# tum-vision/lsd_slam

Hardware: AMD Instinct MI355X
Metric: tracked frames/sec (full track+map loop) at 640x480, frames resident in HBM (8-bit upload excluded: value_pcie_inclusive has it) (higher is better)
Workload: dtype f32

## Files before the change

### include/lsd_slam_hip.hpp

```cpp
#ifndef LSD_SLAM_HIP_HPP
#define LSD_SLAM_HIP_HPP

#include <chrono>
#include <cmath>
#include <cstdint>
#include <cstring>
#include <deque>
#include <exception>
#include <functional>
#include <map>
#include <memory>
#include <mutex>
#include <stdexcept>
#include <string>
#include <tuple>
#include <utility>
#include <vector>

#include "lsdhip.h"

namespace lsd_slam_hip {

struct Error : std::runtime_error {
  int status;
// ... 311 lines not shown
    std::vector<SE3> out((size_t)n);
    for (int j = 0; j < n; j++) out[j] = SE3::from7(results[j].frameToReference);
    return out;
  }
  SE3 trackFrameOnPermaref(Frame* reference, Frame* frame, SE3 referenceToFrame) {
    pushSettings();
    double init[7];
    referenceToFrame.to7(init);
    lsdhip_track_result r;
    check(lsdhip_tracker_track_permaref(h_, reference->permaRef_posData.data(), reference->permaRef_colorAndVarData.data(),
                                        reference->permaRefNumPts, frame->handle(), init, &r), "lsdhip_tracker_track_permaref");
    publish(r);
    return SE3::from7(r.frameToReference);
  }
  void setEnqueueHook(std::function<void()> fn) {
    hook_ = std::move(fn);
    check(lsdhip_tracker_set_enqueue_hook(h_, hook_ ? &SE3Tracker::hookTrampoline : nullptr, this), "lsdhip_tracker_set_enqueue_hook");
  }
  float checkPermaRefOverlap(Frame* reference, SE3 referenceToFrame) {
    double init[7];
    referenceToFrame.to7(init);
    float usage = 0;
    check(lsdhip_tracker_check_overlap(h_, reference->permaRef_posData.data(), reference->permaRefNumPts, init, &usage), "lsdhip_tracker_check_overlap");
    pointUsage = usage;
    return usage;
  }

  float pointUsage = 0, lastGoodCount = 0, lastMeanRes = 0, lastBadCount = 0, lastResidual = 0;
  float affineEstimation_a = 1, affineEstimation_b = 0;
  bool diverged = false, trackingWasGood = false;
  int numEvaluations = 0, numWarpUpdates = 0;
  int levelEvaluations[LSDHIP_PYRAMID_LEVELS] = {0, 0, 0, 0, 0};
  int numLaunches = 0;
  void setSpeculation(int trials, int finestLevelWorkgroups = 0) { check(lsdhip_tracker_set_speculation(h_, trials, finestLevelWorkgroups), "lsdhip_tracker_set_speculation"); }
  void setBatchCoarseMinJobs(int minJobs) { check(lsdhip_tracker_set_batch_coarse_min_jobs(h_, minJobs), "lsdhip_tracker_set_batch_coarse_min_jobs"); }

 private:
  void pushSettings() {
    lsdhip_tracker_settings st;
    st.lambdaSuccessFac = settings.lambdaSuccessFac; st.lambdaFailFac = settings.lambdaFailFac;
    for (int l = 0; l < LSDHIP_PYRAMID_LEVELS; l++) {
      st.lambdaInitial[l] = settings.lambdaInitial[l]; st.stepSizeMin[l] = settings.stepSizeMin[l];
      st.convergenceEps[l] = settings.convergenceEps[l]; st.maxItsPerLvl[l] = settings.maxItsPerLvl[l];
    }
    st.lambdaInitialTestTrack = settings.lambdaInitialTestTrack; st.stepSizeMinTestTrack = settings.stepSizeMinTestTrack;
    st.convergenceEpsTestTrack = settings.convergenceEpsTestTrack; st.maxItsTestTrack = settings.maxItsTestTrack;
    st.huber_d = settings.huber_d; st.var_weight = settings.var_weight;
    check(lsdhip_tracker_set_settings(h_, &st), "lsdhip_tracker_set_settings");
  }
  void publish(const lsdhip_track_result& r) {
    pointUsage = r.pointUsage; lastGoodCount = r.lastGoodCount; lastMeanRes = r.lastMeanRes; lastBadCount = r.lastBadCount;
    lastResidual = r.lastResidual; affineEstimation_a = r.affineEstimation_a; affineEstimation_b = r.affineEstimation_b;
    diverged = r.diverged != 0; trackingWasGood = r.trackingWasGood != 0;
    numEvaluations = r.numEvaluations; numWarpUpdates = r.numWarpUpdates;
    int st[8];
    if (lsdhip_tracker_exec_stats(h_, st) == 0) for (int l = 0; l < LSDHIP_PYRAMID_LEVELS; l++) levelEvaluations[l] = st[3 + l];
    int ls[2];
    if (lsdhip_tracker_launch_stats(h_, ls) == 0) numLaunches = ls[0];
  }
  static void hookTrampoline(void* self) {
    SE3Tracker* t = static_cast<SE3Tracker*>(self);
    try { if (t->hook_) t->hook_(); } catch (...) { t->hookError_ = std::current_exception(); }
  }
  std::function<void()> hook_;
  std::exception_ptr hookError_;
  std::shared_ptr<Context> ctx_;
// ... 126 lines not shown
  float msUpdate = 0, msCreate = 0, msFinalize = 0, msObserve = 0, msRegularize = 0, msPropagate = 0, msFillHoles = 0, msSetDepth = 0;
  lsdhip_depthmap* handle() const { return h_; }

 private:
  void timings() {
    float t[8];
    if (lsdhip_depth_timings(h_, t) == 0) { msUpdate = t[0]; msCreate = t[1]; msFinalize = t[2]; msObserve = t[3]; msRegularize = t[4]; msPropagate = t[5]; msFillHoles = t[6]; msSetDepth = t[7]; }
  }
  std::shared_ptr<Context> ctx_;
  lsdhip_depthmap* h_ = nullptr;
};

class SlamLoop {
 public:
  SlamLoop(int w, int h, const Mat3f& K, const unsigned char* firstImage, bool imagesOnDevice, const float* gtDepth0, int kfEvery)
      : tracker(w, h, K), map(w, h, K), w_(w), h_(h), K_(K), onDevice_(imagesOnDevice), kfEvery_(kfEvery) {
    const int its[LSDHIP_PYRAMID_LEVELS] = {5, 20, 50, 100, 0};
    std::memcpy(tracker.settings.maxItsPerLvl, its, sizeof(its));
    keyframe = makeFrame(0, firstImage);
    if (gtDepth0) {
      keyframe->setDepthFromGroundTruth(gtDepth0);
      map.initializeFromGTDepth(keyframe.get());
    } else {
      map.initializeRandomly(keyframe.get());
    }
    trackKF_ = keyframe;
    reference.importFrame(keyframe.get());
    keyframe->clearDepthHasBeenUpdatedFlag();
    tracker.setEnqueueHook([this]() {
      flushDeferredMapping();
      if (!pendingNext_) return;
      prefetched_ = makeFrame(frameId_ + 1, pendingNext_, true);
      prefetchedSrc_ = pendingNext_;
    });
  }
  SlamLoop(const SlamLoop&) = delete;
  SlamLoop& operator=(const SlamLoop&) = delete;
  void setPipelined(bool on) {
    if (frameId_ != 0) throw Error(LSDHIP_E_STATE, "SlamLoop::setPipelined: switch before the first frame");
    Context::get(w_, h_, K_)->setPipeline(on);
    pipelined_ = on;
  }
  bool pipelined() const { return pipelined_; }
  void flushDeferredMapping() {
    if (!deferredMap_) return;
    std::shared_ptr<Frame> frame = std::move(deferredMap_);
    deferredMap_.reset();
    runUpdate(frame);
  }
  static float keyframeScore(float distanceSquared, float usage) {
    return distanceSquared * 4.0f * 4.0f + (1 - usage) * (1 - usage) * 3.0f * 3.0f;
  }
  std::function<void(Frame&, DepthMap&)> onKeyframeFinished;
  std::function<void(Frame&)> onKeyframeFinishedAsync;
  SE3 step(const unsigned char* image) { return step(image, [](double) {}); }
  template <typename F>
  SE3 step(const unsigned char* image, F&& onTrackEnd, const unsigned char* nextImage = nullptr) {
    if (trackingLost) throw Error(LSDHIP_E_STATE, "SlamLoop: tracking lost (no relocaliser here): create a new loop");
    lsdhip_host_mark(0);
    frameId_++;
    std::shared_ptr<Frame> frame;
    if (prefetched_ && prefetchedSrc_ == image) frame = std::move(prefetched_);
    else frame = makeFrame(frameId_, image);
    prefetched_.reset();
    pendingNext_ = nextImage;
    if (!pipelined_ && keyframe->depthHasBeenUpdatedFlag()) {
      reference.importFrame(keyframe.get());
      keyframe->clearDepthHasBeenUpdatedFlag();
    }
    lsdhip_host_mark(1);
    const std::shared_ptr<Frame> trackedOn = trackKF_;
    SE3 est = tracker.trackFrame(&reference, frame.get(), lastFrameToKF_);
    lsdhip_host_mark(8);
    pendingNext_ = nullptr;
    evaluations += tracker.numEvaluations;
    launches += tracker.numLaunches;
    for (int l = 0; l < LSDHIP_PYRAMID_LEVELS; l++) levelEvaluations[l] += tracker.levelEvaluations[l];
    if (tracker.trackingWasGood) numTrackedGood++;
    numTracked++;
    lastTrackEnd = std::chrono::duration<double>(std::chrono::steady_clock::now().time_since_epoch()).count();
    onTrackEnd(lastTrackEnd);
    if (tracker.diverged || (numKeyframesFinished_ > 5  && !tracker.trackingWasGood)) {
      trackingLost = true;
      reference.invalidate();
      if (map.isValid()) {
        if (mappedOnKF_ >= 5 ) {
          map.finalizeKeyFrame();
          numKeyframesFinished_++;
          if (onKeyframeFinished) onKeyframeFinished(*keyframe, map);
          if (onKeyframeFinishedAsync) onKeyframeFinishedAsync(*keyframe);
        }
        map.invalidate();
      }
      throw Error(LSDHIP_DIVERGED, std::string("SlamLoop: tracking lost at frame ") + std::to_string(frameId_) +
                                       (tracker.diverged ? " (diverged)" : " (trackingWasGood false)"));
    }
// ... 428 lines not shown
```

### include/lsdhip.h

```cpp
#ifndef LSDHIP_H
#define LSDHIP_H

#include <stddef.h>
#include <stdint.h>

#ifdef __cplusplus
extern "C" {
#endif

#define LSDHIP_PYRAMID_LEVELS 5

#define LSDHIP_OK 0
#define LSDHIP_DIVERGED 1
#define LSDHIP_E_ARG (-1)
#define LSDHIP_E_HIP (-2)
#define LSDHIP_E_STATE (-3)
#define LSDHIP_E_CAPACITY (-4)
#define LSDHIP_CLOUD_TABLE_FULL 2
#define LSDHIP_CLOUD_GUARD_POINTS 64

typedef struct lsdhip_ctx lsdhip_ctx;
typedef struct lsdhip_frame lsdhip_frame;
typedef struct lsdhip_tracker lsdhip_tracker;
typedef struct lsdhip_depthmap lsdhip_depthmap;
// ... 78 lines not shown
} lsdhip_track_result;

typedef struct lsdhip_residual_record {
  int warped_size;
  float goodCount, badCount, pointUsage, meanRes, retval;
  float affine_a_lastIt, affine_b_lastIt;
  float weightedError;
  float A[36], b[6], lsError;
  double num_constraints;
} lsdhip_residual_record;

int lsdhip_tracker_create(lsdhip_ctx* ctx, lsdhip_tracker** out);
void lsdhip_tracker_destroy(lsdhip_tracker* t);
int lsdhip_tracker_set_max_its(lsdhip_tracker* t, const int maxItsPerLvl[LSDHIP_PYRAMID_LEVELS]);
typedef struct lsdhip_tracker_settings {
  float lambdaSuccessFac, lambdaFailFac;
  float lambdaInitial[LSDHIP_PYRAMID_LEVELS], stepSizeMin[LSDHIP_PYRAMID_LEVELS], convergenceEps[LSDHIP_PYRAMID_LEVELS];
  int maxItsPerLvl[LSDHIP_PYRAMID_LEVELS];
  float lambdaInitialTestTrack, stepSizeMinTestTrack, convergenceEpsTestTrack, maxItsTestTrack;
  float huber_d, var_weight;
} lsdhip_tracker_settings;
int lsdhip_tracker_get_settings(const lsdhip_tracker* t, lsdhip_tracker_settings* out);
int lsdhip_tracker_set_settings(lsdhip_tracker* t, const lsdhip_tracker_settings* in);
int lsdhip_tracker_exec_stats(const lsdhip_tracker* t, int out[8]);
int lsdhip_tracker_set_speculation(lsdhip_tracker* t, int trials, int finestLevelWorkgroups);
int lsdhip_tracker_set_batch_coarse_min_jobs(lsdhip_tracker* t, int minJobs);
int lsdhip_tracker_launch_stats(const lsdhip_tracker* t, int out[2]);
int lsdhip_tracker_step_stats(const lsdhip_tracker* t, int out[4]);
int lsdhip_tracker_summary_stats(const lsdhip_tracker* t, long long out[6]);
int lsdhip_tracker_eval_throughput(lsdhip_tracker* t, int n, lsdhip_frame** keyframes, lsdhip_frame** frames, const float* refToFrame,
                                   int level, int repeats, double* ms_per_launch, double* bytes_per_launch);
typedef void (*lsdhip_enqueue_hook)(void* user);
int lsdhip_tracker_set_enqueue_hook(lsdhip_tracker* t, lsdhip_enqueue_hook fn, void* user);
int lsdhip_tracker_track(lsdhip_tracker* t, lsdhip_frame* keyframe, lsdhip_frame* frame,
                         const double frameToReference_initialEstimate[7], lsdhip_track_result* out);
int lsdhip_tracker_track_batch(lsdhip_tracker* t, int n, lsdhip_frame** keyframes, lsdhip_frame** frames,
                               const double* frameToReference_initialEstimates, lsdhip_track_result* results);
int lsdhip_tracker_evaluate(lsdhip_tracker* t, lsdhip_frame* keyframe, lsdhip_frame* frame,
                            const float referenceToFrame[7], int level, float affine_a, float affine_b,
                            lsdhip_residual_record* out);
int lsdhip_tracker_evaluate_batch(lsdhip_tracker* t, int n, lsdhip_frame** keyframes, lsdhip_frame** frames,
                                  const float* referenceToFrame, const float* affine, int level, lsdhip_residual_record* out,
                                  int* form);
int lsdhip_tracker_track_permaref(lsdhip_tracker* t, const float* pos3_host, const float* colorAndVar2_host, int n,
                                  lsdhip_frame* frame, const double referenceToFrame[7], lsdhip_track_result* out);
int lsdhip_tracker_track_permaref_batch(lsdhip_tracker* t, int n, const float* pos3_host, const float* colorAndVar2_host,
                                        const int* counts, lsdhip_frame** frames, const double* referenceToFrame,
                                        lsdhip_track_result* results);
int lsdhip_tracker_check_overlap(lsdhip_tracker* t, const float* pos3_host, int n, const double referenceToFrame[7],
                                 float* usage_out);

typedef struct lsdhip_sim3tracker lsdhip_sim3tracker;
typedef struct lsdhip_sim3_result {
  double frameToReference[8];
  float lastResidual, lastDepthResidual, lastPhotometricResidual;
  float pointUsage;
  float affineEstimation_a, affineEstimation_b;
  int diverged;
  int numEvaluations;
  float lastSim3Hessian[49];
} lsdhip_sim3_result;
typedef struct lsdhip_sim3_eval_record {
  int warped_size;
  float pointUsage, affine_a_lastIt, affine_b_lastIt;
  float sumResD, sumResP;
  int numTermsD, numTermsP;
// ... 90 lines not shown
```

### include/lsdhip_driver.h

```cpp
#ifndef LSDHIP_DRIVER_H
#define LSDHIP_DRIVER_H
#include <stdint.h>
#ifdef __cplusplus
extern "C" {
#endif
typedef struct lsdloop lsdloop;
typedef struct lsdloop_stats {
  double seconds_track;
  double seconds_map;
  double seconds_keyframe;
  long long frames;
  long long updates;
  long long keyframes;
  long long evaluations;
  long long tracked_good;
  long long level_evaluations[5];
  long long track_launches;
  long long dropped;
} lsdloop_stats;
int lsdloop_create(int device, int w, int h, const float K4[4], const uint8_t* first_image, int images_on_device,
                   const float* gt_depth0_host, int kf_every, lsdloop** out);
void lsdloop_destroy(lsdloop* l);
int lsdloop_run(lsdloop* l, const uint8_t* const* images, int n, int stop_at_keyframe, double* frameToKeyframe_out);
int lsdloop_get_stats(lsdloop* l, lsdloop_stats* out);
int lsdloop_reset_stats(lsdloop* l);
int lsdloop_copy_keyframe_planes(lsdloop* l, float* idepth_dev, float* idepthVar_dev);
int lsdloop_set_keyframe_ring(lsdloop* l, float* ring_dev, int slots);
long long lsdloop_keyframes_exported(lsdloop* l);
int lsdloop_keep_keyframes(lsdloop* l, int on);
int lsdloop_keyframe_log(lsdloop* l, double* scales_out, long long* points_out, int max);
int lsdloop_set_pipeline(lsdloop* l, int on);
int lsdloop_set_live_queue(lsdloop* l, int frames);
int lsdloop_set_speculation(lsdloop* l, int trials, int finest_level_workgroups);
int lsdloop_observe_time(lsdloop* l, double* ms_out, long long* calls_out);
int lsdloop_observe_work(lsdloop* l, double out3[3]);
int lsdloop_comm_unique_id(unsigned char out128[128]);
int lsdloop_comm_init(lsdloop* l, const unsigned char id128[128], int rank, int world);
int lsdloop_comm_destroy(lsdloop* l);
int lsdloop_gather_keyframes(lsdloop* l, int count, int root, float* recv_dev, long long stride_floats);
int lsdloop_gather_counts(lsdloop* l, int* counts_out, int cap);
int lsdloop_ipc_init(lsdloop* l, int rank, int world, int root, unsigned char handle64_out[64]);
int lsdloop_ipc_connect(lsdloop* l, const unsigned char root_handle64[64]);
int lsdloop_ipc_result(lsdloop* l, int* counts_out, float** data_out);
void* lsdloop_ctx(lsdloop* l);
typedef struct lsdloopbatch lsdloopbatch;
int lsdloopbatch_create(int device, int w, int h, const float K4[4], int S, const uint8_t* const* first_images, int images_on_device,
                        const float* const* gt_depth0_host, int kf_every, lsdloopbatch** out);
void lsdloopbatch_destroy(lsdloopbatch* l);
int lsdloopbatch_run(lsdloopbatch* l, const uint8_t* const* images, int n, double* frameToKeyframe_out);
int lsdloopbatch_get_stats(lsdloopbatch* l, long long* out6_per_sequence);
void* lsdloopbatch_ctx(lsdloopbatch* l);
int lsdloopbatch_set_keyframe_phases(lsdloopbatch* l, const int* phase);
int lsdloopbatch_set_pipeline(lsdloopbatch* l, int on);
int lsdloopbatch_set_coarse_min_jobs(lsdloopbatch* l, int min_jobs);
long long lsdloopbatch_dropped(lsdloopbatch* l, int sequence);
int lsdloopbatch_keep_keyframes(lsdloopbatch* l, int on);
// ... 32 lines not shown
```

### lsd_slam_amd/capi.py

```python
import ctypes as C
import os

import numpy as np

_HERE = os.path.dirname(os.path.abspath(__file__))
LIB_PATH = os.environ.get("LSDHIP_LIB") or os.path.join(_HERE, "liblsdhip.so")
_lib = None

HYP_DTYPE = np.dtype(
    [("isValid", np.uint8), ("_pad", np.uint8, 3), ("blacklisted", np.int32), ("nextStereoFrameMinID", np.float32),
     ("validity_counter", np.int32), ("idepth", np.float32), ("idepth_var", np.float32),
     ("idepth_smoothed", np.float32), ("idepth_var_smoothed", np.float32)])
assert HYP_DTYPE.itemsize == 32


class BuildDefaults(C.Structure):
    _fields_ = [(k, C.c_int) for k in ("ctx_async", "ctx_pipeline", "spec_trials_small", "spec_small_pixels", "spec_trials_mid", "spec_mid_pixels",
                                         "spec_workgroups", "spec_workgroups_above_pixels", "spec_trials_max", "batch_throughput_min_jobs",
                                         "batch_strip_workgroups", "batch_coarse_min_jobs", "batch_coarse_max_pixels",
                                         "batch_coarse_max_points")]


class Params(C.Structure):
    _fields_ = [("minUseGrad", C.c_float), ("cameraPixelNoise2", C.c_float), ("depthSmoothingFactor", C.c_float),
# ... 77 lines not shown
        "lsdhip_frame_set_counters": (i, [vp, i, i, i, i]),
        "lsdhip_frame_depth_updated": (i, [vp]),
        "lsdhip_frame_clear_depth_updated": (i, [vp]),
        "lsdhip_ref_pointcloud": (i, [vp, i, vp, vp, vp, vp]),
        "lsdhip_tracker_create": (i, [vp, pvp]),
        "lsdhip_tracker_destroy": (None, [vp]),
        "lsdhip_tracker_set_max_its": (i, [vp, vp]),
        "lsdhip_tracker_get_settings": (i, [vp, C.POINTER(TrackerSettings)]),
        "lsdhip_tracker_set_settings": (i, [vp, C.POINTER(TrackerSettings)]),
        "lsdhip_depth_copy_rows_batch": (i, [vp, i, vp]),
        "lsdhip_ctx_alloc_dev": (i, [vp, C.c_size_t, vp]),
        "lsdhip_ctx_ipc_export": (i, [vp, vp, vp]),
        "lsdhip_ctx_ipc_open": (i, [vp, vp, vp]),
        "lsdhip_ctx_ipc_close": (i, [vp, vp]),
        "lsdhip_ctx_flag_set": (i, [vp, vp, i]),
        "lsdhip_ctx_flag_wait": (i, [vp, vp, i, vp]),
        "lsdhip_ctx_memset_dev": (i, [vp, vp, i, C.c_size_t]),
        "lsdhip_ctx_read_dev": (i, [vp, vp, vp, C.c_size_t]),
        "lsdhip_ctx_free_dev": (i, [vp, vp]),
        "lsdhip_host_mark": (None, [i]),
        "lsdhip_ctx_aux_begin": (i, [vp]),
        "lsdhip_ctx_aux_end": (i, [vp]),
        "lsdhip_ctx_aux_join": (i, [vp]),
        "lsdhip_ctx_aux_stream": (vp, [vp]),
        "lsdhip_depth_stage_rows": (i, [vp, i, i, i, i]),
        "lsdhip_depth_stage_rows_batch": (i, [vp, i, pvp, C.POINTER(C.c_int), C.POINTER(C.c_int)]),
        "lsdhip_tracker_exec_stats": (i, [vp, vp]),
        "lsdhip_tracker_set_speculation": (i, [vp, i, i]),
        "lsdhip_tracker_set_batch_coarse_min_jobs": (i, [vp, i]),
        "lsdhip_tracker_launch_stats": (i, [vp, vp]),
        "lsdhip_tracker_summary_stats": (i, [vp, vp]),
        "lsdhip_tracker_step_stats": (i, [vp, vp]),
        "lsdhip_tracker_set_enqueue_hook": (i, [vp, vp, vp]),
        "lsdhip_tracker_track": (i, [vp, vp, vp, vp, C.POINTER(TrackResult)]),
        "lsdhip_tracker_track_batch": (i, [vp, i, pvp, pvp, vp, C.POINTER(TrackResult)]),
        "lsdhip_tracker_eval_throughput": (i, [vp, i, pvp, pvp, vp, i, i, C.POINTER(C.c_double), C.POINTER(C.c_double)]),
        "lsdhip_tracker_evaluate": (i, [vp, vp, vp, vp, i, f, f, C.POINTER(ResidualRecord)]),
        "lsdhip_tracker_evaluate_batch": (i, [vp, i, pvp, pvp, vp, vp, i, C.POINTER(ResidualRecord), vp]),
        "lsdhip_tracker_track_permaref": (i, [vp, vp, vp, i, vp, vp, C.POINTER(TrackResult)]),
        "lsdhip_tracker_track_permaref_batch": (i, [vp, i, vp, vp, vp, pvp, vp, C.POINTER(TrackResult)]),
        "lsdhip_tracker_check_overlap": (i, [vp, vp, i, vp, C.POINTER(C.c_float)]),
        "lsdhip_sim3tracker_create": (i, [vp, pvp]),
        "lsdhip_sim3tracker_destroy": (None, [vp]),
        "lsdhip_sim3tracker_set_max_its": (i, [vp, vp]),
        "lsdhip_sim3tracker_track": (i, [vp, vp, vp, vp, i, i, C.POINTER(Sim3Result)]),
        "lsdhip_sim3tracker_track_batch": (i, [vp, i, pvp, pvp, vp, i, i, C.POINTER(Sim3Result)]),
        "lsdhip_host_se3f_step": (i, [vp, vp, vp]),
        "lsdhip_host_ldlt6": (i, [vp, vp, vp]),
        "lsdhip_host_sim3_step": (i, [vp, vp, vp]),
        "lsdhip_host_ldlt7": (i, [vp, vp, vp]),
        "lsdhip_devtest_se3f_lm_step": (i, [vp, i, vp, vp, vp, vp, vp, vp]),
        "lsdhip_devtest_sim3_lm_step": (i, [vp, i, vp, vp, vp, vp, vp, vp, vp]),
        "lsdhip_sim3tracker_evaluate": (i, [vp, vp, vp, vp, i, f, f, C.POINTER(Sim3EvalRecord)]),
        "lsdhip_depth_create": (i, [vp, pvp]),
        "lsdhip_depth_destroy": (None, [vp]),
        "lsdhip_depth_is_valid": (i, [vp]),
        "lsdhip_depth_invalidate": (i, [vp]),
        "lsdhip_depth_reset": (i, [vp]),
        "lsdhip_depth_init_gt": (i, [vp, vp]),
        "lsdhip_depth_init_random": (i, [vp, vp]),
        "lsdhip_depth_set_from_existing": (i, [vp, vp]),
        "lsdhip_depth_update": (i, [vp, pvp, i]),
        "lsdhip_depth_observe_work": (i, [vp, vp]),
        "lsdhip_depth_update_batch": (i, [i, pvp, pvp]),
        "lsdhip_depth_create_keyframe": (i, [vp, vp, C.POINTER(C.c_float)]),
        "lsdhip_depth_change_keyframe_batch": (i, [i, pvp, pvp, C.POINTER(C.c_float)]),
# ... 56 lines not shown
```

### lsd_slam_amd/csrc/lsdhip_internal.hpp

```cpp
#pragma once
#include <hip/hip_runtime.h>
#include <cmath>
#include <cstddef>
#include <cstdint>
#include <cstdio>
#include <cstring>
#include <mutex>
#include <string>
#include <vector>
#include "../../include/lsdhip.h"

#define LSD_LEVELS LSDHIP_PYRAMID_LEVELS
#define LSD_TRACK_MIN_LEVEL 1
#define LSD_TRACK_MAX_LEVEL 5
#define LSD_QUICK_KF_CHECK_LVL 4

void lsd_set_error(const char* fmt, ...);
#define HIPCHK(expr)                                                                       \
  do {                                                                                     \
    hipError_t e_ = (expr);                                                                \
    if (e_ != hipSuccess) {                                                                \
      lsd_set_error("%s failed: %s (%s:%d)", #expr, hipGetErrorString(e_), __FILE__, __LINE__); \
      return LSDHIP_E_HIP;                                                                 \
    }                                                                                      \
// ... 10 lines not shown
  RS_M = 0,
  RS_GOOD, RS_BAD, RS_SUMRES2, RS_SUMSIGNED, RS_SXX, RS_SYY, RS_SX, RS_SY, RS_SW, RS_USAGE,
  RS_WERR,
  RS_A0,
  RS_B0 = RS_A0 + 21,
  RS_ERR = RS_B0 + 6,
  RS_NREF,
  RS_END,
  RS_TOP0 = RS_END
};
static_assert(RS_TOP0 + 3 <= RS_NUM, "record too small");
static_assert(RS_END <= RS_NUM, "record too small");

struct TrackLevel {
  const float* kf_idepth;
  const float* kf_idepthVar;
  const float* kf_image;
  const uint8_t* kf_refBlk;
  const float4* fr_grad;
  const float* pts_pos;
  const float* pts_colvar;
  int npts;
  int w, h;
  int nblocks;
  int singlePass;
  int tilePx;
  float fx, fy, cx, cy, fxi, fyi, cxi, cyi;
  float lambdaInitial, stepSizeMin, convergenceEps;
  int maxIts;
  float minWarped;
  int writeMask;
};

struct TrackJob {
  TrackLevel lv[LSD_LEVELS];
  uint8_t* wasGood;
  float cameraPixelNoise2, var_weight, huber_half;
  float lambdaSuccessFac, lambdaFailFac;
  int useAffine;
  int lastLevel;
  int topLevel;
  lsdm::SE3fH T0;
  float aff_a0, aff_b0;
  int evalOnly;
  int trackFrameSemantics;
};
struct TrackSpec {
  int specC;
  int specGrid;
  int trials[LSD_LEVELS];
  uint8_t* wasGoodSide;
  unsigned maskStride;
  int seq;
  int copyMask;
  unsigned long long dbgCum;
  unsigned long long* dbgCounters;
  int last;
#ifdef LSD_PHASE_TRACE
  int traceWg;
#endif
#ifdef LSD_DEVTOOLS
  int* dbgLog;
#endif
};

#define LSD_SPEC_MAX 6
struct TrackState {
  lsdm::SE3fH T;
  lsdm::SE3fH Tn;
  float R[9], t[3];
  float aff_a, aff_b, aff_a_lastIt, aff_b_lastIt;
  float lastErr, LM_lambda, last_residual;
  int level, iteration, incTry, phase;
  int pending;
  float A[36], b[6];
  float inc[6];
  float bytes;
  int done, diverged;
  int numEvaluations, numWarpUpdates;
  float pointUsage, goodCount, badCount, meanRes;
  int levelEvals[LSD_LEVELS];
  int ncand;
  int lastCand;
  int numLaunches;
};

struct TrackSummary {
  int done;
  int diverged, level, numEvaluations, numWarpUpdates, pad_[3];
  float q[4], t[3];
  float lastResidual, pointUsage, goodCount, badCount, meanRes, aff_a, aff_b, aff_a_lastIt, aff_b_lastIt;
  float sums[RS_NUM];
  double bytes;
  int levelEvals[LSD_LEVELS];
  int numLaunches;
  int lastCand;
  int seq;
  int exhausted;
  unsigned check;
};
#define LSD_SUMMARY_CHECK_WORDS (offsetof(TrackSummary, seq) / 4)
__host__ __device__ static inline unsigned lsd_summary_term(unsigned i, unsigned bits) { return bits * (2u * i + 1u); }

struct DeferredSlot { double sum, count, flag, pad; };
#define LSD_NUM_SLOTS 256
#define LSD_DEFAULT_ASYNC 0
#define LSD_DEFAULT_PIPELINE 0
#define LSD_SPEC_TRIALS_SMALL 6
#define LSD_SPEC_SMALL_PX 6144
#define LSD_SPEC_TRIALS_MID 5
#define LSD_SPEC_MID_PX 90112
#define LSD_SPEC_CAP_WORKGROUPS 80
#define LSD_SPEC_CAP_ABOVE_PX 24576
#ifndef LSD_OBS_SPLIT_MIN_MAPS
#define LSD_OBS_SPLIT_MIN_MAPS 4
#endif
#define LSD_OBS_WALK_WAVES 4096
#define LSD_BATCH_THROUGHPUT_MIN_JOBS 8
#define LSD_BATCH_SPEC_MAX 4
#define LSD_BATCH_SPEC_PIXELS 500000
#define LSD_BATCH_STRIP_WORKGROUPS 768
struct lsdhip_frame;

#define LSD_CTX_LOCK(c) std::lock_guard<std::recursive_mutex> lsd_ctx_lock_((c)->mtx)
struct lsdhip_ctx {
  std::recursive_mutex mtx;
  int device = 0;
  bool async = LSD_DEFAULT_ASYNC != 0;
  DeferredSlot* h_slots = nullptr;
// ... 136 lines not shown
  int levelEvaluations[LSD_LEVELS] = {};
  int block = 256;
  int grid_cap = 304;
  int recent[4] = {0, 0, 0, 0};
  int specC = 6;
  int soloMinJobs = -1;
  bool specAuto = true;
  int specCaps[LSD_LEVELS] = {0, 0, 0, 0, 0};
  int specLevel[LSD_LEVELS] = {0, 0, 0, 0, 0};
  int specCap = LSD_SPEC_CAP_WORKGROUPS;
  uint8_t* d_maskSide = nullptr;
  int maskSet = 0;
  long long maskMergeSeq[2] = {0, 0};
  size_t maskStride = 0;
  int numLaunches = 0;
  long long sumPolled = 0, sumLate = 0, sumLateMaxNs = 0, sumLateWords = 0;
  int sumLateFirstWord = -1, sumLateLastWord = -1;
  unsigned long long dbgCum = 0;
  std::vector<unsigned> dumpL0;
  unsigned long long* d_dbg = nullptr;
#ifdef LSD_DEVTOOLS
  int* d_log = nullptr;
  std::vector<int> lastLog;
#endif
  TrackSpec spec = {};
  const lsdhip_frame* jobKf = nullptr;
  unsigned jobKfVersion = 0;
  int jobTag = 0, launchOrdinal = 0;
  int budgetExtra = 2;
  int budgetFixed = 0;
  long long dbgJobs = 0, dbgEnqueued = 0, dbgMisses = 0, dbgWaitNs = 0, dbgLaunchNs = 0;
  TrackSummary* h_summary = nullptr;
  TrackSummary* d_summary = nullptr;
  unsigned long long* d_trace = nullptr;
  int batch_capacity = 0;
  TrackJob* d_bjobs = nullptr;
  TrackJob* h_bjobs = nullptr;
  TrackState* d_bstate = nullptr;
  float* d_bscratch = nullptr;
  int batchRecent[4] = {0, 0, 0, 0};
  int batchTag = 1;
  TrackSummary* h_bsummary = nullptr;
  float* d_pts = nullptr;
  int pts_capacity = 0;
};

#ifdef __HIP_DEVICE_COMPILE__
#define LSD_G __attribute__((address_space(1)))
#else
#define LSD_G
#endif
template <typename T> __host__ __device__ inline LSD_G T* lsd_g(T* p) { return (LSD_G T*)p; }
struct HypPlanes {
  LSD_G uint8_t* valid;
  LSD_G int32_t* blacklisted;
  LSD_G float* nextID;
  LSD_G int32_t* validity;
  LSD_G float* idepth;
  LSD_G float* var;
  LSD_G float* idepth_s;
  LSD_G float* var_s;
};

struct StereoRef {
  LSD_G const float* image;
  LSD_G const uint8_t* wasGood;
// ... 115 lines not shown
```

### lsd_slam_amd/csrc/pose_math.hpp

```cpp
#pragma once
#include <hip/hip_runtime.h>
#include <cmath>

#define LSDM_HD __host__ __device__ inline

namespace lsdm {
struct Quatd { double w, x, y, z; };
struct Quatf { float w, x, y, z; };
struct SE3dH { Quatd q; double t[3]; };
struct SE3fH { Quatf q; float t[3]; };
struct Sim3dH { Quatd q; double t[3]; double s; };

template <typename Q> LSDM_HD Q q_conj(const Q& a) { Q r = {a.w, -a.x, -a.y, -a.z}; return r; }
template <typename Q> LSDM_HD Q q_mul(const Q& a, const Q& b) {
  Q r;
  r.w = a.w * b.w - a.x * b.x - a.y * b.y - a.z * b.z;
  r.x = a.w * b.x + a.x * b.w + a.y * b.z - a.z * b.y;
  r.y = a.w * b.y + a.y * b.w + a.z * b.x - a.x * b.z;
  r.z = a.w * b.z + a.z * b.w + a.x * b.y - a.y * b.x;
  return r;
}
LSDM_HD void q_normalize(Quatf& q) {
  float n = sqrtf(q.x * q.x + q.y * q.y + q.z * q.z + q.w * q.w);
  q.w /= n; q.x /= n; q.y /= n; q.z /= n;
// ... 22 lines not shown
LSDM_HD void quatf_to_rot(const Quatf& q, float R[9]) { q_to_rot<Quatf, float>(q, R); }
LSDM_HD void quatd_to_rot(const Quatd& q, double R[9]) { q_to_rot<Quatd, double>(q, R); }

LSDM_HD SE3dH se3d_from7(const double p[7]) { SE3dH T; T.q = {p[0], p[1], p[2], p[3]}; T.t[0] = p[4]; T.t[1] = p[5]; T.t[2] = p[6]; return T; }
LSDM_HD void se3d_to7(const SE3dH& T, double p[7]) { p[0] = T.q.w; p[1] = T.q.x; p[2] = T.q.y; p[3] = T.q.z; p[4] = T.t[0]; p[5] = T.t[1]; p[6] = T.t[2]; }
LSDM_HD SE3dH se3d_inverse(const SE3dH& T) {
  SE3dH r;
  r.q = q_conj(T.q);
  double nt[3] = {T.t[0] * -1.0, T.t[1] * -1.0, T.t[2] * -1.0};
  q_rotate<Quatd, double>(r.q, nt, r.t);
  return r;
}
LSDM_HD SE3fH se3f_from_d(const SE3dH& T) {
  SE3fH r;
  r.q = {(float)T.q.w, (float)T.q.x, (float)T.q.y, (float)T.q.z};
  q_normalize(r.q);
  for (int i = 0; i < 3; i++) r.t[i] = (float)T.t[i];
  return r;
}
LSDM_HD SE3dH se3d_from_f(const SE3fH& T) {
  SE3dH r;
  r.q = {(double)T.q.w, (double)T.q.x, (double)T.q.y, (double)T.q.z};
  q_normalize(r.q);
  for (int i = 0; i < 3; i++) r.t[i] = (double)T.t[i];
  return r;
}
LSDM_HD SE3fH se3f_inverse(const SE3fH& T) {
  SE3fH r;
  r.q = q_conj(T.q);
  float nt[3] = {T.t[0] * -1.0f, T.t[1] * -1.0f, T.t[2] * -1.0f};
  q_rotate<Quatf, float>(r.q, nt, r.t);
  return r;
}
LSDM_HD SE3fH se3f_mul(const SE3fH& a, const SE3fH& b) {
  SE3fH r = a;
  float rt[3];
  q_rotate<Quatf, float>(a.q, b.t, rt);
  for (int i = 0; i < 3; i++) r.t[i] = a.t[i] + rt[i];
  r.q = q_mul(a.q, b.q);
  q_normalize(r.q);
  return r;
}
LSDM_HD SE3fH se3f_exp(const float a[6]) {
  const float eps = static_cast<float>(1e-5);
  float ox = a[3], oy = a[4], oz = a[5];
  float theta_sq = ox * ox + (oy * oy + oz * oz);
  float theta = sqrtf(theta_sq);
  float half_theta = 0.5f * theta;
  float imag, real;
  if (theta < eps) {
    float theta_po4 = theta_sq * theta_sq;
    imag = 0.5f - static_cast<float>(1.0 / 48.0) * theta_sq + static_cast<float>(1.0 / 3840.0) * theta_po4;
    real = 1.0f - 0.5f * theta_sq + static_cast<float>(1.0 / 384.0) * theta_po4;
  } else {
    float s = sinf(half_theta);
    imag = s / theta;
    real = cosf(half_theta);
  }
  SE3fH r;
  r.q = {real, imag * ox, imag * oy, imag * oz};
  q_normalize(r.q);
  float Om[9] = {0, -oz, oy, oz, 0, -ox, -oy, ox, 0};
  float Om2[9];
  for (int i = 0; i < 3; i++)
    for (int j = 0; j < 3; j++) {
      float acc = Om[i * 3 + 0] * Om[0 * 3 + j];
// ... 80 lines not shown
```

### lsd_slam_amd/csrc/track_device.hpp

```cpp
#pragma once
#include "lsdhip_internal.hpp"
#include <type_traits>

template <int CTRL, int ROW_MASK, int BANK_MASK>
__device__ __forceinline__ float dpp_f(float v) {
  return __builtin_bit_cast(float, __builtin_amdgcn_update_dpp(0, __builtin_bit_cast(int, v), CTRL, ROW_MASK, BANK_MASK, true));
}
__device__ __forceinline__ int dpp_max_i(int a, int b) { return a > b ? a : b; }
template <int CTRL, int ROW_MASK, int BANK_MASK>
__device__ __forceinline__ int dpp_i(int v) {
  return __builtin_amdgcn_update_dpp(-1, v, CTRL, ROW_MASK, BANK_MASK, false);
}
template <int CTRL, int ROW_MASK, int BANK_MASK>
__device__ __forceinline__ int dpp_i0(int v) {
  return __builtin_amdgcn_update_dpp(0, v, CTRL, ROW_MASK, BANK_MASK, true);
}
__device__ __forceinline__ int wave_max_to_lane63(int v) {
  int t = dpp_max_i(v, dpp_i<0x111, 0xf, 0xf>(v));
  t = dpp_max_i(t, dpp_i<0x112, 0xf, 0xf>(v));
  t = dpp_max_i(t, dpp_i<0x113, 0xf, 0xf>(v));
  t = dpp_max_i(t, dpp_i<0x114, 0xf, 0xe>(t));
  t = dpp_max_i(t, dpp_i<0x118, 0xf, 0xc>(t));
  t = dpp_max_i(t, dpp_i<0x142, 0xa, 0xf>(t));
  t = dpp_max_i(t, dpp_i<0x143, 0xc, 0xf>(t));
// ... 298 lines not shown
__device__ __forceinline__ lsdm::SE3fH se3f_mul_wave(const lsdm::SE3fH& a, const lsdm::SE3fH& b, const int lane) {
  lsdm::SE3fH r = a;
  float rt[3];
  lsdm::q_rotate<lsdm::Quatf, float>(a.q, b.t, rt);
#pragma unroll
  for (int i = 0; i < 3; i++) r.t[i] = a.t[i] + rt[i];
  r.q = lsdm::q_mul(a.q, b.q);
  q_normalize_wave(r.q, lane);
  return r;
}

__device__ __forceinline__ void write_summary(const TrackState& s, const float* tot, TrackSummary* out, const int doneWord) {
  unsigned chk = (unsigned)doneWord;
#define SUM_PUT_I(field, value) do { const int v_ = (value); out->field = v_; chk += lsd_summary_term((unsigned)(offsetof(TrackSummary, field) / 4), (unsigned)v_); } while (0)
#define SUM_PUT_F(field, value) do { const float v_ = (value); out->field = v_; chk += lsd_summary_term((unsigned)(offsetof(TrackSummary, field) / 4), __float_as_uint(v_)); } while (0)
#define SUM_PUT_IA(field, i, value) do { const int v_ = (value); out->field[i] = v_; chk += lsd_summary_term((unsigned)(offsetof(TrackSummary, field) / 4 + (i)), (unsigned)v_); } while (0)
#define SUM_PUT_FA(field, i, value) do { const float v_ = (value); out->field[i] = v_; chk += lsd_summary_term((unsigned)(offsetof(TrackSummary, field) / 4 + (i)), __float_as_uint(v_)); } while (0)
  SUM_PUT_I(diverged, s.diverged); SUM_PUT_I(level, s.level); SUM_PUT_I(numEvaluations, s.numEvaluations); SUM_PUT_I(numWarpUpdates, s.numWarpUpdates);
  SUM_PUT_IA(pad_, 0, 0); SUM_PUT_IA(pad_, 1, 0); SUM_PUT_IA(pad_, 2, 0);
  SUM_PUT_FA(q, 0, s.T.q.w); SUM_PUT_FA(q, 1, s.T.q.x); SUM_PUT_FA(q, 2, s.T.q.y); SUM_PUT_FA(q, 3, s.T.q.z);
  SUM_PUT_FA(t, 0, s.T.t[0]); SUM_PUT_FA(t, 1, s.T.t[1]); SUM_PUT_FA(t, 2, s.T.t[2]);
  SUM_PUT_F(lastResidual, s.last_residual); SUM_PUT_F(pointUsage, s.pointUsage); SUM_PUT_F(goodCount, s.goodCount); SUM_PUT_F(badCount, s.badCount);
  SUM_PUT_F(meanRes, s.meanRes); SUM_PUT_F(aff_a, s.aff_a); SUM_PUT_F(aff_b, s.aff_b); SUM_PUT_F(aff_a_lastIt, s.aff_a_lastIt); SUM_PUT_F(aff_b_lastIt, s.aff_b_lastIt);
  for (int i = 0; i < RS_NUM; i++) SUM_PUT_FA(sums, i, tot[i]);
  {
    const double b = (double)s.bytes;
    out->bytes = b;
    const unsigned long long u = (unsigned long long)__double_as_longlong(b);
    chk += lsd_summary_term((unsigned)(offsetof(TrackSummary, bytes) / 4), (unsigned)u) + lsd_summary_term((unsigned)(offsetof(TrackSummary, bytes) / 4 + 1), (unsigned)(u >> 32));
  }
  for (int l = 0; l < LSD_LEVELS; l++) SUM_PUT_IA(levelEvals, l, s.levelEvals[l]);
  SUM_PUT_I(numLaunches, s.numLaunches);
  SUM_PUT_I(lastCand, s.lastCand);
#undef SUM_PUT_I
#undef SUM_PUT_F
#undef SUM_PUT_IA
#undef SUM_PUT_FA
  out->check = chk;
  __threadfence_system();
  out->done = doneWord;
}

struct LmShared {
  float gj[48];
  float tot[RS_NUM];
};
struct LmPar {
  float lambdaInitial, stepSizeMin, convergenceEps, minWarped, lambdaSuccessFac, lambdaFailFac;
  int maxIts, w, h, writeMask, evalOnly, useAffine, tfSemantics, lastLevel, trials;
};
__device__ __forceinline__ void stage_lm_par(const TrackJob& job, int level, LmPar& p, const int trials = 1) {
  const TrackLevel& L = job.lv[level];
  LmPar v;
  v.lambdaInitial = L.lambdaInitial; v.stepSizeMin = L.stepSizeMin; v.convergenceEps = L.convergenceEps; v.minWarped = L.minWarped;
  v.lambdaSuccessFac = job.lambdaSuccessFac; v.lambdaFailFac = job.lambdaFailFac;
  v.maxIts = L.maxIts; v.w = L.w; v.h = L.h; v.writeMask = L.writeMask; v.evalOnly = job.evalOnly; v.useAffine = job.useAffine;
  v.tfSemantics = job.trackFrameSemantics; v.lastLevel = job.lastLevel;
  v.trials = trials;
  p = v;
}

#ifdef LSD_PHASE_TRACE
#define LM_MARK(k) do { if (trp && lane == 0) trp[k] = clock64(); } while (0)
#else
#define LM_MARK(k) do { } while (0)
#endif
__device__ __forceinline__ float lm_werr(float sumWeightedErr, int M) { return sumWeightedErr * frcp((float)((M >> 2) << 2)); }
__device__ __forceinline__ float lm_lambda_fail(float LM_lambda, int incTry, float lambdaFailFac) {
  if (LM_lambda == 0) return 0.2f;
  double p = 1.0;
  for (int i = 0; i < incTry; i++) p *= (double)lambdaFailFac;
  return (float)((double)LM_lambda * p);
}
template <bool SPEC = false>
__device__ __forceinline__ bool lm_wave(const LmPar& par, TrackState& S, const float col, float* tot, const int lane,
                                        TrackSummary* out, unsigned long long* trp, const int consumed = 0, const int mycand = 0, const int doneWord = 1) {
  float* const s_gj = tot - 48;
  S.lastCand = consumed;
  S.ncand = 1;
  const LmPar L = par;
  const int maxIts = L.maxIts;
  const int M = (int)rl(col, RS_M);
  const float refNum = rl(col, RS_NREF);
  const float goodCount = rl(col, RS_GOOD), badCount = rl(col, RS_BAD);
  float aff_a_lastIt, aff_b_lastIt;
  {
    const float sxx = rl(col, RS_SXX), syy = rl(col, RS_SYY), sx = rl(col, RS_SX), sy = rl(col, RS_SY), sw = rl(col, RS_SW);
    const float isw = frcp(sw);
    aff_a_lastIt = fsqrt((syy - sy * sy * isw) * frcp(sxx - sx * sx * isw));
    aff_b_lastIt = (sy - aff_a_lastIt * sx) * isw;
  }
// ... 75 lines not shown
  }
  if (start_iteration && iteration < maxIts) { S.numWarpUpdates = S.numWarpUpdates + 1; incTry = 0; propose = true; }
  S.lastErr = lastErr;
  S.LM_lambda = LM_lambda;
  S.iteration = iteration;
  LM_MARK(13);
  if (propose) {
    const int extra = SPEC ? mycand : 0;
    for (int j = 0; j < extra; j++) { incTry++; LM_lambda = lm_lambda_fail(LM_lambda, incTry, L.lambdaFailFac); }
    S.ncand = L.trials;
    float inc[6];
    const float damp = 1 + LM_lambda;
    LM_MARK(14);
    gj6_solve_wave(S.A, S.b, damp, s_gj, lane, inc);
    LM_MARK(15);
    S.incTry = incTry + 1;
#pragma unroll
    for (int i = 0; i < 6; i++) S.inc[i] = inc[i];
    const lsdm::SE3fH Tn = se3f_mul_wave(se3f_exp_wave(inc, lane), T, lane);
    S.Tn = Tn;
    float R[9];
    lsdm::quatf_to_rot(Tn.q, R);
#pragma unroll
    for (int i = 0; i < 9; i++) S.R[i] = R[i];
    S.t[0] = Tn.t[0]; S.t[1] = Tn.t[1]; S.t[2] = Tn.t[2];
    S.phase = 1;
    LM_MARK(16);
    return true;
  }
  S.incTry = incTry;
  if (!tfSemantics) S.last_residual = lastErr;
  if (S.level == L.lastLevel) {
    S.done = 1;
    if (out && lane == 0) write_summary(S, tot, out, doneWord);
  } else {
    S.level = S.level - 1;
    S.phase = 0;
    S.Tn = T;
    float R[9];
    lsdm::quatf_to_rot(T.q, R);
#pragma unroll
    for (int i = 0; i < 9; i++) S.R[i] = R[i];
    S.t[0] = T.t[0]; S.t[1] = T.t[1]; S.t[2] = T.t[2];
  }
  return false;
}

__device__ __forceinline__ void accumulate_point(const PointOut& o, float (&acc)[RS_END]) {
  acc[RS_M] += 1.f;
  acc[RS_SXX] = __builtin_fmaf(o.c1 * o.c1, o.hw, acc[RS_SXX]);
  acc[RS_SYY] = __builtin_fmaf(o.c2 * o.c2, o.hw, acc[RS_SYY]);
  acc[RS_SX] = __builtin_fmaf(o.c1, o.hw, acc[RS_SX]);
  acc[RS_SY] = __builtin_fmaf(o.c2, o.hw, acc[RS_SY]);
  acc[RS_SW] += o.hw;
  if (o.good) { acc[RS_GOOD] += 1.f; acc[RS_SUMRES2] = __builtin_fmaf(o.res, o.res, acc[RS_SUMRES2]); acc[RS_SUMSIGNED] += o.res; }
  else acc[RS_BAD] += 1.f;
  acc[RS_USAGE] += o.usage;
  acc[RS_WERR] += o.werr;
#pragma unroll
  for (int r = 0; r < 6; r++) {
    float Jw = o.J[r] * o.w;
#pragma unroll
    for (int c = r; c < 6; c++) acc[tri_index(r, c)] = __builtin_fmaf(Jw, o.J[c], acc[tri_index(r, c)]);
  }
  float resw = o.res * o.w;
#pragma unroll
  for (int r = 0; r < 6; r++) acc[RS_B0 + r] = __builtin_fmaf(resw, o.J[r], acc[RS_B0 + r]);
  acc[RS_ERR] = __builtin_fmaf(resw, o.res, acc[RS_ERR]);
}

__device__ __forceinline__ void make_ctx_dev(const TrackJob& jobr, const TrackState& S, int level, EvalCtx& a) {
  const TrackJob* job = &jobr;
  const TrackLevel& L = job->lv[level];
  a.kf_idepth = (gfloat*)L.kf_idepth; a.kf_idepthVar = (gfloat*)L.kf_idepthVar; a.kf_image = (gfloat*)L.kf_image; a.fr_grad = (gfloat*)L.fr_grad;
  a.pts_pos = (gfloat*)L.pts_pos; a.pts_colvar = (gfloat*)L.pts_colvar; a.npts = L.npts; a.w = L.w; a.h = L.h;
  a.fx = L.fx; a.fy = L.fy; a.cx = L.cx; a.cy = L.cy; a.fxi = L.fxi; a.fyi = L.fyi; a.cxi = L.cxi; a.cyi = L.cyi;
#pragma unroll
  for (int i = 0; i < 9; i++) a.R[i] = S.R[i];
#pragma unroll
  for (int i = 0; i < 3; i++) a.t[i] = S.t[i];
  a.aff_a = S.aff_a; a.aff_b = S.aff_b;
  a.cameraPixelNoise2 = job->cameraPixelNoise2; a.var_weight = job->var_weight; a.huber_half = job->huber_half;
}

template <int N>
__device__ __forceinline__ void copy_words(void* dst, const void* src, int tid, int nthreads) {
  const unsigned* s = (const unsigned*)src;
  unsigned* d = (unsigned*)dst;
  for (int i = tid; i < N; i += nthreads) d[i] = s[i];
}

__device__ __forceinline__ int xcd_tile(int b, int nb) { return (nb & 7) == 0 ? (b & 7) * (nb >> 3) + (b >> 3) : b; }


#define RS_COLS 44
struct TrackScratch {
  float* sums;
  int4* topkey;
  float* topval;
  int max_rows;
  int cmax;
  float* recs;
#ifdef LSD_PHASE_TRACE
  unsigned long long* trace;
#endif
};
```

### lsd_slam_amd/csrc/tracker.hip

```cpp
#include <atomic>
#include <chrono>
#include "track_device.hpp"


#ifdef LSD_PHASE_TRACE
#define PHASE_MARK(k) do { if (trOn_ && threadIdx.x == 0) tr_[k] = clock64(); } while (0)
#define LSD_TRACE_WORDS 32
#else
#define PHASE_MARK(k) do { } while (0)
#endif

#ifdef LSD_DEVTOOLS
#define LAUNCH_LOG(exitCode, pendingIn, ncandIn, pcUsed) do { \
    if (!BATCH && MODE == TS_FUSED && blockIdx.x == 0 && threadIdx.x == 0 && spec.dbgLog && spec.seq != 0) { \
      int* lg_ = spec.dbgLog + ((spec.seq & 0xFFF) * 16); \
      lg_[0] = spec.seq; lg_[1] = (exitCode); lg_[2] = parity | (first << 1) | (spec.last << 2); lg_[3] = lvlIn_; lg_[4] = (pendingIn); lg_[5] = (ncandIn); \
      lg_[6] = (pcUsed); lg_[7] = S.level; lg_[8] = S.numEvaluations; lg_[9] = S.numLaunches; lg_[10] = S.done; lg_[11] = S.phase; lg_[12] = S.incTry; \
      lg_[13] = S.ncand; lg_[14] = S.pending; lg_[15] = numLaunchesIn_; } } while (0)
#else
#define LAUNCH_LOG(exitCode, pendingIn, ncandIn, pcUsed) do { } while (0)
#endif

enum { TS_FUSED = 0, TS_LM = 1, TS_EVAL = 2 };
__device__ __forceinline__ void track_state_begin(TrackState& S, const TrackJob& job, const int tid) {
  if (tid == 0) {
    S.T = job.T0;
    set_eval_pose(S, job.T0);
    S.aff_a = job.aff_a0; S.aff_b = job.aff_b0; S.aff_a_lastIt = job.aff_a0; S.aff_b_lastIt = job.aff_b0;
    S.lastErr = 0; S.LM_lambda = 0; S.last_residual = 0;
    S.level = job.topLevel; S.iteration = 0; S.incTry = 0; S.phase = 0; S.pending = 0;
    S.done = 0; S.diverged = 0; S.numEvaluations = 0; S.numWarpUpdates = 0;
    S.pointUsage = 0; S.goodCount = 0; S.badCount = 0; S.meanRes = 0;
    S.bytes = 0;
    for (int l = 0; l < LSD_LEVELS; l++) S.levelEvals[l] = 0;
    S.ncand = 1; S.lastCand = 0; S.numLaunches = 0;
  }
  if (tid < 36) S.A[tid] = 0;
  if (tid < 6) { S.b[tid] = 0; S.inc[tid] = 0; }
}
__device__ __forceinline__ void tail_row(const PointOut& o, float* row) {
  row[0] = o.werr;
  int k = 1;
#pragma unroll
  for (int rr = 0; rr < 6; rr++) {
    const float Jw = o.J[rr] * o.w;
#pragma unroll
    for (int cc = rr; cc < 6; cc++) row[k++] = Jw * o.J[cc];
  }
  const float resw = o.res * o.w;
#pragma unroll
  for (int rr = 0; rr < 6; rr++) row[k++] = resw * o.J[rr];
  row[k++] = resw * o.res;
}

template <int BLOCK, bool BATCH, int MODE>
__device__ __forceinline__ void track_step_impl(const TrackJob& jobv, const TrackJob* __restrict__ jobs, TrackState* __restrict__ st2,
                                                TrackScratch sc, TrackSummary* __restrict__ out, int parity, int first, const TrackSpec& spec) {
  const TrackJob& job = BATCH ? jobs[blockIdx.y] : jobv;
  unsigned warm = 0;
  if (!BATCH) {
// ... 33 lines not shown
  const bool leader = blockIdx.x == 0;
  const int cmax = sc.cmax;
  TrackState* next = st2 + (1 - parity);
  const int outp = MODE == TS_EVAL ? parity : 1 - parity;
  const float* sums_in0 = sc.sums + (size_t)parity * cmax * RS_COLS * max_rows;
  float* sums_out = sc.sums + (size_t)outp * cmax * RS_COLS * max_rows;
  const int4* topkey_in0 = sc.topkey + (size_t)parity * cmax * max_rows;
  int4* topkey_out = sc.topkey + (size_t)outp * cmax * max_rows;
  const float* topval_in0 = sc.topval + (size_t)parity * cmax * max_rows * 96;
  float* topval_out = sc.topval + (size_t)outp * cmax * max_rows * 96;
  constexpr int NSLOT = 16;
  constexpr int TRIALS_MAX = BATCH ? (MODE == TS_EVAL ? 1 : LSD_BATCH_SPEC_MAX) : LSD_SPEC_MAX;
  constexpr bool SPEC_LM = MODE != TS_EVAL;
  static_assert(TRIALS_MAX * (NSLOT * RS_COLS + 96 + 1) <= CPP * (BLOCK + 1) + 8, "the finishing phase's tables must fit the reduction buffer");
  float (*const s_sumT)[NSLOT][RS_COLS] = (float (*)[NSLOT][RS_COLS])s_red;
  float (*const s_subT)[3][32] = (float (*)[3][32])(s_red + TRIALS_MAX * NSLOT * RS_COLS);
  int* const s_nsubT = (int*)(s_red + TRIALS_MAX * (NSLOT * RS_COLS + 96));
  __shared__ float s_rec[TRIALS_MAX][32];
#ifdef LSD_PHASE_TRACE
  __shared__ unsigned long long* s_trp;
  unsigned long long* tr_ = sc.trace;
  const bool trOn_ = sc.trace != nullptr && (int)blockIdx.x == (BATCH ? spec.traceWg : 0) && (!BATCH || blockIdx.y == 0);
  if (trOn_ && tid == 0) {
    unsigned long long n = sc.trace[0];
    sc.trace[0] = n + 1;
    tr_ = sc.trace + 1 + (n % 4096) * LSD_TRACE_WORDS;
    for (int k = 0; k < LSD_TRACE_WORDS; k++) tr_[k] = 0;
    tr_[8] = wall_clock64();
    tr_[24] = (unsigned long long)gridDim.x; tr_[25] = (unsigned long long)gridDim.y;
    s_trp = tr_;
  }
#endif
  PHASE_MARK(0);
  if (!BATCH && MODE == TS_FUSED && !first && !leader && st2[parity].done) return;
  if (!BATCH && MODE == TS_FUSED && leader && tid == 0 && spec.seq != 0) out->seq = spec.seq;
  if (first) {
    track_state_begin(S, job, tid);
  } else {
    copy_words<sizeof(TrackState) / 4>(&S, st2 + parity, tid, BLOCK);
    if (SPEC_LM && cmax > 1 && tid < 32 * TRIALS_MAX) (&s_rec[0][0])[tid] = sc.recs[(size_t)parity * cmax * 32 + (tid < 32 * cmax ? tid : 0)];
  }
  __syncthreads();
  PHASE_MARK(1);
#ifdef LSD_DEVTOOLS
  const int lvlIn_ = S.level, numLaunchesIn_ = S.numLaunches, pendingIn_ = S.pending, ncandIn_ = S.ncand;
  int pcLog_ = -1;
#endif
  if (S.done) {
    LAUNCH_LOG(1, pendingIn_, ncandIn_, -1);
    if (MODE != TS_EVAL && leader) { copy_words<sizeof(TrackState) / 4>(next, &S, tid, BLOCK); }
    return;
  }
  const int lvlPending = S.level;
  const int doneWord = (MODE == TS_FUSED && spec.seq != 0) ? (BATCH ? spec.seq : (spec.seq >> 12)) : 1;
  if (MODE == TS_FUSED) {
    const int nbl = job.lv[lvlPending].nblocks;
    const int tr = (spec.specC > 1 && spec.trials[lvlPending] > 1) ? spec.trials[lvlPending] : 1;
    cand = (int)blockIdx.x / nbl;
    bx = (int)blockIdx.x - cand * nbl;
    const bool needTrial = S.pending ? cand < tr : cand == 0;
    const bool needNext = S.pending && lvlPending > job.lastLevel && (int)blockIdx.x < job.lv[lvlPending - 1].nblocks;
    if (!leader && !needTrial && !needNext) return;
  }

  if (BATCH && MODE == TS_LM) {
    cand = (int)blockIdx.x;
    bx = 0;
    const int tr = (spec.specC > 1 && spec.trials[lvlPending] > 1) ? spec.trials[lvlPending] : 1;
    if (!leader && !(S.pending && cand < tr)) return;
  }
  if (BATCH && MODE == TS_EVAL) {
    const int nbl = job.lv[lvlPending].nblocks;
    cand = (int)blockIdx.x / nbl;
    bx = (int)blockIdx.x - cand * nbl;
  }

  constexpr int CHMAX = 8;
  int cntv = 0;
  unsigned ow[CHMAX];
  auto strip_request = [&](const int lvl, const int tile_) {
    const TrackLevel& L = job.lv[lvl];
    const int px = L.w * L.h;
    const int base_ = tile_ * L.tilePx;
    const int b0_ = base_ >> 8;
    const int mblk_ = (min(base_ + L.tilePx, px) - base_ + 255) >> 8;
    const gbyte* offs = (const gbyte*)L.kf_refBlk;
    const __attribute__((address_space(1))) int* cnts = (const __attribute__((address_space(1))) int*)(offs + ((size_t)((px + 255) >> 8) << 8));
// ... 64 lines not shown
          const float* tv = topval_in0 + (size_t)ca * max_rows * 96;
          if (keysA[rj] >= 0) a0 = tv[(size_t)srcA[rj] * 32 + j];
          if (rj == 0 && keysA[2] >= 0) a2 = tv[(size_t)srcA[2] * 32 + j];
        }
        if (cb >= 0) {
          merge(kvb, keysB, srcB);
          if (single && j < 29) {
            const float* tv = topval_in0 + (size_t)cb * max_rows * 96;
            if (keysB[rj] >= 0) b0 = tv[(size_t)srcB[rj] * 32 + j];
            if (rj == 0 && keysB[2] >= 0) b2 = tv[(size_t)srcB[2] * 32 + j];
          }
        }
        if (lane == 0) {
          s_nsubT[ca] = (keysA[0] >= 0) + (keysA[1] >= 0) + (keysA[2] >= 0);
          if (cb >= 0) s_nsubT[cb] = (keysB[0] >= 0) + (keysB[1] >= 0) + (keysB[2] >= 0);
        }
        if (single) {
          if (j < 29) {
            if (keysA[rj] >= 0) s_subT[ca][rj][j] = a0;
            if (rj == 0 && keysA[2] >= 0) s_subT[ca][2][j] = a2;
            if (cb >= 0) {
              if (keysB[rj] >= 0) s_subT[cb][rj][j] = b0;
              if (rj == 0 && keysB[2] >= 0) s_subT[cb][2][j] = b2;
            }
          }
        } else {
          const bool second = lane >= 3;
          const int r = second ? lane - 3 : lane;
          const int c = second ? cb : ca;
          int key = -1;
          if (lane < 6 && c >= 0) key = second ? (r == 0 ? keysB[0] : (r == 1 ? keysB[1] : keysB[2])) : (r == 0 ? keysA[0] : (r == 1 ? keysA[1] : keysA[2]));
          if (key >= 0) {
            EvalCtx a;
            make_ctx_dev(job, S, level, a);
            if (c > 0) {
              const float* rec = s_rec[c];
#pragma unroll
              for (int i = 0; i < 9; i++) a.R[i] = rec[13 + i];
#pragma unroll
              for (int i = 0; i < 3; i++) a.t[i] = rec[22 + i];
            }
            const int idx = (a.npts >= 0) ? key : ((key / a.h) + (key % a.h) * a.w);
            float px, py, pz, I_ref, var;
            int maskIdx;
            fetch_point(a, idx, px, py, pz, I_ref, var, maskIdx);
            PointOut o;
            eval_point(a, px, py, pz, I_ref, var, o);
            float* sub = s_subT[c][r];
            sub[0] = o.werr;
            int k = 1;
#pragma unroll
            for (int rr = 0; rr < 6; rr++) {
              float Jw = o.J[rr] * o.w;
#pragma unroll
              for (int cc = rr; cc < 6; cc++) sub[k++] = Jw * o.J[cc];
            }
            float resw = o.res * o.w;
#pragma unroll
            for (int rr = 0; rr < 6; rr++) sub[k++] = resw * o.J[rr];
            sub[k++] = resw * o.res;
          }
        }
      };
      auto tail_rows = [&](const int ca, const int cb, auto nqn) {
        constexpr int NQ = decltype(nqn)::value;
        const int cbb = cb < 0 ? ca : cb;
        const float4* ta = (const float4*)(topval_in0 + (size_t)ca * max_rows * 96);
// ... 25 lines not shown
            const int owner = own ? (int)__ffsll((long long)own) - 1 : 0;
            const int row = __builtin_amdgcn_readlane(e0, owner);
            if (k0 == m && m >= 0) { k0 = k1; e0 = e1; k1 = k2; e1 = e2; k2 = -1; }
            if (m >= 0) {
              nsub++;
              const int qsel = row >> 3;
#pragma unroll
              for (int q = 0; q < NQ; q++) {
                if (q == qsel) {
                  float4 w4 = v[q];
                  asm volatile("" : "+v"(w4.x), "+v"(w4.y), "+v"(w4.z), "+v"(w4.w));
                  if ((lane >> 3) == (row & 7)) *(float4*)&s_subT[c][r][(lane & 7) * 4] = w4;
                }
              }
            }
          }
          if (lane == 0) s_nsubT[c] = nsub;
        };
        pick(va, ca);
        if (cb >= 0) pick(vb, cb);
      };
    auto wave_tail = [&]() {
      const int ca = WAVES - 1 - wave;
      const int cb = ca + WAVES < ncandPending ? ca + WAVES : -1;
      if (ca < ncandPending) {
        if (BATCH && job.lv[level].tilePx > 0 && nb <= 24) {
          if (nb <= 5) tail_rows(ca, cb, std::integral_constant<int, 2>());
          else if (nb <= 13) tail_rows(ca, cb, std::integral_constant<int, 5>());
          else tail_rows(ca, cb, std::integral_constant<int, 9>());
        } else if (nb <= 128) tail_two(ca, cb, std::integral_constant<int, 2>());
        else tail_two(ca, cb, std::integral_constant<int, 5>());
      }
    };
    if (tid == SUMW * 64 - 1) stage_lm_par(job, level, s_par, (spec.specC > 1 && spec.trials[level] > 1) ? spec.trials[level] : 1);
    if (wave < SUMW) {
      const int t = tid;
      const int slot_ = t / (RS_COLS / 4);
      const bool sumLane = slot_ < NSLOT;
      const int slot = sumLane ? slot_ : 0, c4 = sumLane ? t - slot_ * (RS_COLS / 4) : 0;
      {
        const int K = (nb + NSLOT - 1) / NSLOT;
        const float4* p = (const float4*)sums_in0 + c4;
        const size_t trialStrideF4 = (size_t)RS_COLS * max_rows / 4;
        auto colsum = [&](auto qn, auto ntn, const int base) {
          constexpr int Q = decltype(qn)::value, NT = decltype(ntn)::value;
          float4 v[NT][Q];
#pragma unroll
          for (int c = 0; c < NT; c++) {
            const int pc = base + c < ncandPending ? base + c : ncandPending - 1;
            const float4* pp = p + (size_t)pc * trialStrideF4;
#pragma unroll
            for (int q = 0; q < Q; q++) {
              const int r = slot + NSLOT * q;
              v[c][q] = pp[(size_t)(r < nb ? r : slot) * (RS_COLS / 4)];
            }
          }
#pragma unroll
          for (int c = 0; c < NT; c++) {
            float4 a4 = make_float4(0.f, 0.f, 0.f, 0.f);
#pragma unroll
            for (int q = 0; q < Q; q++) {
              const bool live = q < K && slot + NSLOT * q < nb;
              a4.x += live ? v[c][q].x : 0.f;
              a4.y += live ? v[c][q].y : 0.f;
              a4.z += live ? v[c][q].z : 0.f;
              a4.w += live ? v[c][q].w : 0.f;
            }
// ... 78 lines not shown
        for (int k = 1; k < NSLOT; k++) Mf += s_sumT[pc][k][RS_M];
        float s = 0.f;
        if (tid < RS_END) {
          s = s_sumT[pc][0][tid];
#pragma unroll
          for (int k = 1; k < NSLOT; k++) s += s_sumT[pc][k][tid];
        }
        const int M = (int)Mf;
        int need = M & 3;
        if (need > s_nsubT[pc]) need = s_nsubT[pc];
        const int subIdx = (tid == RS_WERR) ? 0 : ((tid >= RS_A0 && tid < RS_B0) ? 1 + tid - RS_A0 : ((tid >= RS_B0 && tid < RS_ERR) ? 22 + tid - RS_B0 : (tid == RS_ERR ? 28 : -1)));
        const float sub0 = s_subT[pc][0][subIdx < 0 ? 0 : subIdx], sub1 = s_subT[pc][1][subIdx < 0 ? 0 : subIdx], sub2 = s_subT[pc][2][subIdx < 0 ? 0 : subIdx];
        if (subIdx >= 0) {
          if (need > 0) s -= sub0;
          if (need > 1) s -= sub1;
          if (need > 2) s -= sub2;
        }
        if (tid < RS_NUM) sh.tot[tid] = s;
#ifdef LSD_ORDER_CHECK
        if (!BATCH && spec.dbgCounters) {
          unsigned hv = tid < RS_END ? __float_as_uint(s) * (2654435761u * (unsigned)(tid + 1)) : 0u;
          hv += (unsigned)pc * 97u;
          for (int off = 32; off > 0; off >>= 1) hv += __shfl_xor(hv, off);
          if (tid == 0) {
            const unsigned long long slot = 8 + 2 * ((spec.dbgCum / 400ull) % 8192ull);
            __hip_atomic_fetch_min(&spec.dbgCounters[slot], (unsigned long long)hv, __ATOMIC_RELAXED, __HIP_MEMORY_SCOPE_AGENT);
            __hip_atomic_fetch_max(&spec.dbgCounters[slot + 1], (unsigned long long)hv, __ATOMIC_RELAXED, __HIP_MEMORY_SCOPE_AGENT);
          }
        }
#endif
        PHASE_MARK(3);
#ifdef LSD_PHASE_TRACE
        if (trOn_ && tid == 0) { tr_[19] = (unsigned long long)ncandPending; tr_[7] = (unsigned long long)pc; }
        lm_wave<SPEC_LM>(s_par, S, s, sh.tot, tid, leader ? out : nullptr, trOn_ ? tr_ : nullptr, pc, cand, doneWord);
#else
        lm_wave<SPEC_LM>(s_par, S, s, sh.tot, tid, leader ? out : nullptr, nullptr, pc, cand, doneWord);
#endif
      }
    }
    __syncthreads();
    PHASE_MARK(4);
    if (S.done) {
      if (!BATCH && MODE == TS_FUSED && S.lastCand > 0 && spec.copyMask != 0 && job.lv[level].writeMask && cand == 0 && bx < nb) {
        const uint8_t* side = spec.wasGoodSide + (size_t)(S.lastCand - 1) * spec.maskStride;
        EvalCtx a;
        make_ctx_dev(job, S, level, a);
        const int work = a.npts >= 0 ? a.npts : a.w * a.h;
        for (int i = bx * BLOCK + tid; i < work; i += nb * BLOCK) {
          float px, py, pz, I_ref, var;
          int maskIdx;
          if (fetch_point(a, i, px, py, pz, I_ref, var, maskIdx) && maskIdx >= 0) job.wasGood[maskIdx] = side[maskIdx];
        }
      }
      if (leader) copy_words<sizeof(TrackState) / 4>(next, &S, tid, BLOCK);
      LAUNCH_LOG(2, pendingIn_, ncandIn_, S.lastCand);
      return;
    }
    if (cand > 0 && bx == 0 && S.phase == 1 && cand < S.ncand && tid < 25) {
      float v;
      if (tid < 6) v = S.inc[tid];
      else if (tid < 13) v = ((const float*)&S.Tn)[tid - 6];
      else if (tid < 22) v = S.R[tid - 13];
      else v = S.t[tid - 22];
      sc.recs[((size_t)outp * cmax + cand) * 32 + tid] = v;
    }
  }

  if (MODE == TS_LM) {
    __syncthreads();
    if (tid == 0) { S.pending = 1; S.numLaunches = S.numLaunches + 1; }
    __syncthreads();
    if (leader) copy_words<sizeof(TrackState) / 4>(next, &S, tid, BLOCK);
    return;
  }

  const int level = S.level;
  const int nb = job.lv[level].nblocks;
  if (MODE == TS_FUSED && level != lvlPending) { cand = 0; bx = (int)blockIdx.x; }
  if (bx >= nb || cand >= S.ncand) return;
  sums_out += (size_t)cand * RS_COLS * max_rows;
  topkey_out += (size_t)cand * max_rows;
  topval_out += (size_t)cand * max_rows * 96;
  const int tile = xcd_tile(bx, nb);
  EvalCtx a;
  make_ctx_dev(job, S, level, a);
  if (BATCH && MODE == TS_EVAL && cand > 0) {
    const float* rec = sc.recs + ((size_t)parity * cmax + cand) * 32;
#pragma unroll
    for (int i = 0; i < 9; i++) a.R[i] = rec[13 + i];
#pragma unroll
    for (int i = 0; i < 3; i++) a.t[i] = rec[22 + i];
  }
  gbyte* wasGood = (gbyte*)(job.lv[level].writeMask ? (cand == 0 ? job.wasGood : spec.wasGoodSide + (size_t)(cand - 1) * spec.maskStride) : nullptr);
  const int work = a.npts >= 0 ? a.npts : a.w * a.h;
  float acc[RS_END];
#pragma unroll
  for (int k = 0; k < RS_END; k++) acc[k] = 0.f;
  int key0 = -1, key1 = -1, key2 = -1;

  if (BATCH && job.lv[level].tilePx > 0) {
    unsigned* s_list = (unsigned*)s_red;
    const int tilePx = job.lv[level].tilePx;
    const int base = tile * tilePx;
    const int stripEnd = min(base + tilePx, work);
    const int b0 = base >> 8;
    const int mblk = (stripEnd - base + 255) >> 8;
    const float inv_w = 1.0f / (float)a.w;
    if (!(havePre && level == lvlPending)) strip_request(level, tile);
    int incl = cntv + dpp_i0<0x111, 0xf, 0xf>(cntv);
    incl += dpp_i0<0x112, 0xf, 0xf>(cntv);
    incl += dpp_i0<0x113, 0xf, 0xf>(cntv);
    incl += dpp_i0<0x114, 0xf, 0xe>(incl);
    incl += dpp_i0<0x118, 0xf, 0xc>(incl);
    incl += dpp_i0<0x142, 0xa, 0xf>(incl);
    const int total = __builtin_amdgcn_readlane(incl, 31);
    const int waveU = __builtin_amdgcn_readfirstlane(wave);
    PHASE_MARK(20);
#pragma unroll
    for (int c = 0; c < CHMAX; c++) {
      const int blk = c * 4 + waveU;
      if (blk < mblk) {
        const int cb = __builtin_amdgcn_readlane(cntv, blk);
        const int pb = __builtin_amdgcn_readlane(incl, blk) - cb;
#pragma unroll
        for (int k = 0; k < 4; k++) {
          const int sl = lane + 64 * k;
// ... 144 lines not shown
    __syncthreads();
    if (stripRows && hp == 0 && candLane) {
      float* row = topval_out + (size_t)(tile * 3 + (tid - (BLOCK - 64))) * 32;
      if (cKey >= 0) {
        PointOut o;
        eval_finish(a, cq, ct, cPz, cImg, cVar, o);
        tail_row(o, row);
      }
      ((int*)row)[31] = cKey;
    }
    if (tid < CPP && hp * CPP + tid < RS_END) {
      float s = s_sum[0][tid];
#pragma unroll
      for (int sl = 1; sl < RSLICE; sl++) s += s_sum[sl][tid];
      sums_out[(size_t)tile * RS_COLS + (hp * CPP + tid)] = s;
    }
  }
  if (!stripRows) block_top3(key0, key1, key2, s_wtop, s_top);
  if (tid == 0) topkey_out[tile] = make_int4(s_top[0], s_top[1], s_top[2], -1);
  if (job.lv[level].singlePass && key0 >= 0) {
    const int r = key0 == s_top[0] ? 0 : (key0 == s_top[1] ? 1 : (key0 == s_top[2] ? 2 : -1));
    if (r >= 0) {
      float* dst = topval_out + (size_t)(tile * 3 + r) * 32;
      dst[0] = acc[RS_WERR];
#pragma unroll
      for (int k = 0; k < 21; k++) dst[1 + k] = acc[RS_A0 + k];
#pragma unroll
      for (int k = 0; k < 6; k++) dst[22 + k] = acc[RS_B0 + k];
      dst[28] = acc[RS_ERR];
    }
  }
  if (MODE == TS_FUSED && leader) copy_words<sizeof(TrackState) / 4>(next, &S, tid, BLOCK);
 
  if (MODE == TS_FUSED && leader && tid == 0 && spec.last != 0) out->exhausted = spec.seq;
  LAUNCH_LOG(3, pendingIn_, ncandIn_, S.lastCand);
  PHASE_MARK(6);
#ifdef LSD_PHASE_TRACE
  if (trOn_ && tid == 0) tr_[9] = wall_clock64();
#endif
}

template <int BLOCK, bool BATCH, int MODE = TS_FUSED>
__global__ __launch_bounds__(BLOCK) void k_track_step(TrackJob jobv, const TrackJob* __restrict__ jobs, TrackState* __restrict__ st2,
                                                       TrackScratch sc, TrackSummary* __restrict__ out, int parity, int first, TrackSpec spec) {
#ifdef LSD_ORDER_CHECK
  if (!BATCH && spec.dbgCounters && threadIdx.x == 0) {
    const unsigned long long fin = __hip_atomic_load(&spec.dbgCounters[0], __ATOMIC_RELAXED, __HIP_MEMORY_SCOPE_AGENT);
    if (fin < spec.dbgCum) {
      __hip_atomic_fetch_add(&spec.dbgCounters[1], 1ull, __ATOMIC_RELAXED, __HIP_MEMORY_SCOPE_AGENT);
      __hip_atomic_fetch_max(&spec.dbgCounters[2], spec.dbgCum - fin, __ATOMIC_RELAXED, __HIP_MEMORY_SCOPE_AGENT);
    }
  }
#endif
  track_step_impl<BLOCK, BATCH, MODE>(jobv, jobs, st2, sc, out, parity, first, spec);
#ifdef LSD_ORDER_CHECK
  __syncthreads();
  if (!BATCH && spec.dbgCounters && threadIdx.x == 0) __hip_atomic_fetch_add(&spec.dbgCounters[0], 1ull, __ATOMIC_RELEASE, __HIP_MEMORY_SCOPE_AGENT);
#endif
}

#define LSD_SOLO_MAX_PX 4800
#define LSD_SOLO_TRIPS 9
#define LSD_SOLO_MAX_PTS (LSD_SOLO_TRIPS * 512)
#define LSD_SOLO_LDS_PTS 4544
static_assert(LSD_SOLO_LDS_PTS <= LSD_SOLO_MAX_PTS, "every point of the LDS lists has a register slot");
constexpr int lsd_solo_max_interior() {
  int best = 0;
  for (int w = 3; w <= LSD_SOLO_MAX_PX / 3; w++) {
    const int h = LSD_SOLO_MAX_PX / w;
    if ((w - 2) * (h - 2) > best) best = (w - 2) * (h - 2);
  }
  return best;
}
static_assert(lsd_solo_max_interior() <= LSD_SOLO_LDS_PTS, "the dense interior of any level k_track_solo takes fits its LDS lists");
#define LSD_SOLO_MIN_JOBS 24
template <int BLOCK>
__global__ __launch_bounds__(BLOCK) void k_track_solo(const TrackJob* __restrict__ jobs, TrackState* __restrict__ st2, TrackSummary* __restrict__ outs,
                                                          const int parity, const int doneWord) {
  const TrackJob& job = jobs[blockIdx.x];
  st2 += 2 * (size_t)blockIdx.x;
  TrackSummary* out = outs + blockIdx.x;
  constexpr int WAVES = BLOCK / 64;
  constexpr int HALF = BLOCK / 2;
  constexpr int CPP = RS_END;
  constexpr int RSLICE = BLOCK / CPP;
  constexpr int RRUN = (HALF + RSLICE - 1) / RSLICE;
  constexpr int TRIPS = LSD_SOLO_TRIPS;
  static_assert(WAVES * 3 <= 64, "top-3 merge in one wave");
  static_assert((size_t)TRIPS * BLOCK * 4 <= sizeof(float) * (CPP * (HALF + 1) + RRUN), "the level's list borrows the reduction buffer");
  __shared__ TrackState S;
  __shared__ LmShared sh;
  __shared__ LmPar s_par;
  __shared__ __attribute__((aligned(16))) float s_red[CPP * (HALF + 1) + RRUN];
  __shared__ float s_sum[RSLICE][64];
  __shared__ float s_sub[3][32];
  __shared__ int s_wtop[WAVES][3];
  __shared__ v4f s_tex[LSD_SOLO_MAX_PX];
  __shared__ float s_var[LSD_SOLO_LDS_PTS], s_img[LSD_SOLO_LDS_PTS];
  const int tid = threadIdx.x, wave = tid >> 6, lane = tid & 63;
  track_state_begin(S, job, tid);
  __syncthreads();
  int listLevel = -1, total = 0;
  EvalCtx a;
  unsigned pXY[TRIPS];
  float pZ[TRIPS];
  auto taps = [&](const PointWarp& q, const bool fetch, PointTexels& t) {
    const int ix = fetch ? (int)q.u_new : 0;
    const int iy = fetch ? (int)q.v_new : 0;
    const v4f* bp = s_tex + (ix + __mul24(iy, a.w));
    const v4f v00 = bp[0], v10 = bp[1], v01 = bp[a.w], v11 = bp[a.w + 1];
    t.t00 = Texel3{v00.x, v00.y, v00.z}; t.t10 = Texel3{v10.x, v10.y, v10.z};
    t.t01 = Texel3{v01.x, v01.y, v01.z}; t.t11 = Texel3{v11.x, v11.y, v11.z};
  };
  for (int guard = 0; guard < 4096; guard++) {
    const int level = S.level;
    if (S.done) break;
    const TrackLevel& L = job.lv[level];
    const int work = L.w * L.h;
    if (L.tilePx <= 0 || work > LSD_SOLO_MAX_PX || L.writeMask) break;
    if (level != listLevel) {
      make_ctx_dev(job, S, level, a);
      if (tid == BLOCK - 1) stage_lm_par(job, level, s_par, 1);
      const int mblk = (work + 255) >> 8;
      const gbyte* offs = (const gbyte*)L.kf_refBlk;
      const __attribute__((address_space(1))) int* cnts = (const __attribute__((address_space(1))) int*)(offs + ((size_t)mblk << 8));
      const int cntv = lane < mblk ? cnts[lane] : 0;
      int incl = cntv + dpp_i0<0x111, 0xf, 0xf>(cntv);
      incl += dpp_i0<0x112, 0xf, 0xf>(cntv);
      incl += dpp_i0<0x113, 0xf, 0xf>(cntv);
      incl += dpp_i0<0x114, 0xf, 0xe>(incl);
      incl += dpp_i0<0x118, 0xf, 0xc>(incl);
      incl += dpp_i0<0x142, 0xa, 0xf>(incl);
      total = __builtin_amdgcn_readlane(incl, 31);
// ... 302 lines not shown
    int v[LSD_LEVELS] = {0, 0, 0, 0, 0};
    sscanf(e, "%d,%d,%d,%d,%d", &v[0], &v[1], &v[2], &v[3], &v[4]);
    for (int l = 0; l < LSD_LEVELS; l++) t->specCaps[l] = v[l] < 0 ? 0 : (v[l] & ~7);
  }
  if (const char* e = getenv("LSDHIP_SPEC_LEVELS")) {
    int v[LSD_LEVELS] = {0, 0, 0, 0, 0};
    sscanf(e, "%d,%d,%d,%d,%d", &v[0], &v[1], &v[2], &v[3], &v[4]);
    for (int l = 0; l < LSD_LEVELS; l++) t->specLevel[l] = v[l] < 0 ? 0 : (v[l] > LSD_SPEC_MAX ? LSD_SPEC_MAX : v[l]);
  }
  t->maskStride = (((size_t)c->wl[LSD_TRACK_MIN_LEVEL] * c->hl[LSD_TRACK_MIN_LEVEL]) + 255) & ~(size_t)255;
  HIPCHK(hipMalloc((void**)&t->d_maskSide, 2 * t->maskStride * (LSD_SPEC_MAX - 1)));
  HIPCHK(hipMemsetAsync(t->d_maskSide, 0, 2 * t->maskStride * (LSD_SPEC_MAX - 1), c->stream));
  HIPCHK(hipMalloc((void**)&t->d_partials, partials_bytes));
  HIPCHK(hipMemsetAsync(t->d_partials, 0, partials_bytes, c->stream));
#ifdef LSD_ORDER_CHECK
  {
    const size_t nd = 8 + 2 * 8192;
    HIPCHK(hipMalloc((void**)&t->d_dbg, nd * 8));
    std::vector<unsigned long long> init(nd, 0);
    for (size_t i = 8; i < nd; i += 2) init[i] = ~0ull;
    HIPCHK(hipMemcpy(t->d_dbg, init.data(), nd * 8, hipMemcpyHostToDevice));
  }
#endif
#ifdef LSD_DEVTOOLS
  HIPCHK(hipMalloc((void**)&t->d_log, 4096 * 16 * 4));
  HIPCHK(hipMemset(t->d_log, 0, 4096 * 16 * 4));
#endif
  HIPCHK(hipMalloc((void**)&t->d_state, 2 * sizeof(TrackState)));
  HIPCHK(hipMemsetAsync(t->d_state, 0, 2 * sizeof(TrackState), c->stream));
#ifdef LSD_PHASE_TRACE
  HIPCHK(hipMalloc((void**)&t->d_trace, (1 + 4096 * LSD_TRACE_WORDS) * 8));
  HIPCHK(hipMemsetAsync(t->d_trace, 0, (1 + 4096 * LSD_TRACE_WORDS) * 8, c->stream));
#endif
  HIPCHK(hipHostMalloc((void**)&t->h_summary, sizeof(TrackSummary), hipHostMallocMapped));
  HIPCHK(hipHostGetDevicePointer((void**)&t->d_summary, t->h_summary, 0));
  memset(t->h_summary, 0, sizeof(TrackSummary));
  const char* env = getenv("LSDHIP_HOST_LM");
  t->hostLM = env && env[0] == '1';
  if (const char* e = getenv("LSDHIP_SPIN")) t->spinWait = e[0] != '0';
  if (const char* e = getenv("LSDHIP_BUDGET_EXTRA")) { t->budgetExtra = atoi(e); if (t->budgetExtra < 1) t->budgetExtra = 1; }
  if (const char* e = getenv("LSDHIP_BUDGET_FIXED")) { t->budgetFixed = atoi(e); if (t->budgetFixed < 1) t->budgetFixed = 0; }
  *out = t;
  return LSDHIP_OK;
}
extern "C" void lsdhip_tracker_destroy(lsdhip_tracker* t) {
  if (!t) return;
  {
    lsdhip_ctx* c = t->ctx;
    LSD_CTX_LOCK(c);
    for (size_t i = 0; i < c->pendingMerges.size();)
      if (c->pendingMerges[i].doneSeq == &t->maskMergeSeq[0] || c->pendingMerges[i].doneSeq == &t->maskMergeSeq[1]) c->pendingMerges.erase(c->pendingMerges.begin() + i);
      else i++;
  }
#ifdef LSD_DEVTOOLS
  if (getenv("LSDHIP_TRACK_DEBUG") && t->dbgJobs > 0)
    fprintf(stderr, "TRACKDBG jobs %lld launches enqueued %.2f/job, budget misses %lld, host launch %.1f us/job, host wait %.1f us/job\n", t->dbgJobs,
            (double)t->dbgEnqueued / t->dbgJobs, t->dbgMisses, t->dbgLaunchNs / 1e3 / t->dbgJobs, t->dbgWaitNs / 1e3 / t->dbgJobs);
#endif
  (void)hipSetDevice(t->ctx->device);
  (void)hipStreamSynchronize(t->ctx->stream);
#ifdef LSD_ORDER_CHECK
  {
    std::vector<unsigned long long> h(8 + 2 * 8192, 0);
    (void)hipMemcpy(h.data(), t->d_dbg, h.size() * 8, hipMemcpyDeviceToHost);
    int used = 0, split = 0;
    for (size_t i = 8; i < h.size(); i += 2) if (h[i] != ~0ull) { used++; if (h[i] != h[i + 1]) split++; }
    if (const char* path = getenv("LSDHIP_ORDER_DUMP")) {
      if (FILE* f = fopen(path, "w")) {
        for (size_t i = 8; i < h.size(); i += 2) if (h[i] != ~0ull) fprintf(f, "%zu %llx %llx\n", (i - 8) / 2, h[i], h[i + 1]);
        fclose(f);
      }
    }
    fprintf(stderr, "ORDERCHECK: %llu workgroups finished (%llu launched), %llu started before every earlier workgroup had finished (largest deficit %llu); "
                    "%d launch slots hashed, %d in which the workgroups did NOT all see the same totals\n", h[0], t->dbgCum, h[1], h[2], used, split);
  }
#endif
  if (t->d_dbg) (void)hipFree(t->d_dbg);
#ifdef LSD_PHASE_TRACE
  if (const char* path = getenv("LSDHIP_TRACE_FILE")) {
    std::vector<unsigned long long> h(1 + 4096 * LSD_TRACE_WORDS);
    if (hipMemcpy(h.data(), t->d_trace, h.size() * 8, hipMemcpyDeviceToHost) == hipSuccess) {
      if (FILE* f = fopen(path, "w")) {
        unsigned long long n = h[0] < 4096 ? h[0] : 4096;
        for (unsigned long long i = 0; i < n; i++) {
          for (int k = 0; k < LSD_TRACE_WORDS; k++) fprintf(f, "%llu ", h[1 + i * LSD_TRACE_WORDS + k]);
          fprintf(f, "\n");
        }
        fclose(f);
      }
    }
  }
  (void)hipFree(t->d_trace);
#endif
  if (t->d_bjobs) { (void)hipFree(t->d_bjobs); (void)hipFree(t->d_bstate); (void)hipFree(t->d_bscratch); (void)hipHostFree(t->h_bjobs); (void)hipHostFree(t->h_bsummary); }
  (void)hipFree(t->d_partials);
  (void)hipFree(t->d_maskSide);
  (void)hipFree(t->d_state);
#ifdef LSD_DEVTOOLS
  (void)hipFree(t->d_log);
#endif
  (void)hipHostFree(t->h_summary);
  if (t->d_pts) (void)hipFree(t->d_pts);
  delete t;
}
extern "C" int lsdhip_tracker_set_enqueue_hook(lsdhip_tracker* t, lsdhip_enqueue_hook fn, void* user) {
  if (!t) return LSDHIP_E_ARG;
  t->enqueueHook = fn;
  t->enqueueHookUser = user;
  return LSDHIP_OK;
}
extern "C" int lsdhip_tracker_get_settings(const lsdhip_tracker* t, lsdhip_tracker_settings* o) {
  if (!t || !o) return LSDHIP_E_ARG;
  o->lambdaSuccessFac = t->lambdaSuccessFac; o->lambdaFailFac = t->lambdaFailFac;
  for (int l = 0; l < LSD_LEVELS; l++) {
    o->lambdaInitial[l] = t->lambdaInitial[l]; o->stepSizeMin[l] = t->stepSizeMin[l]; o->convergenceEps[l] = t->convergenceEps[l];
    o->maxItsPerLvl[l] = t->maxItsPerLvl[l];
  }
  o->lambdaInitialTestTrack = t->lambdaInitialTestTrack; o->stepSizeMinTestTrack = t->stepSizeMinTestTrack;
  o->convergenceEpsTestTrack = t->convergenceEpsTestTrack; o->maxItsTestTrack = t->maxItsTestTrack;
  o->huber_d = t->huber_d; o->var_weight = t->var_weight;
  return LSDHIP_OK;
}
extern "C" int lsdhip_tracker_set_settings(lsdhip_tracker* t, const lsdhip_tracker_settings* in) {
  if (!t || !in) return LSDHIP_E_ARG;
  t->lambdaSuccessFac = in->lambdaSuccessFac; t->lambdaFailFac = in->lambdaFailFac;
  for (int l = 0; l < LSD_LEVELS; l++) {
    t->lambdaInitial[l] = in->lambdaInitial[l]; t->stepSizeMin[l] = in->stepSizeMin[l]; t->convergenceEps[l] = in->convergenceEps[l];
    t->maxItsPerLvl[l] = in->maxItsPerLvl[l];
  }
  t->lambdaInitialTestTrack = in->lambdaInitialTestTrack; t->stepSizeMinTestTrack = in->stepSizeMinTestTrack;
  t->convergenceEpsTestTrack = in->convergenceEpsTestTrack; t->maxItsTestTrack = in->maxItsTestTrack;
  t->huber_d = in->huber_d; t->var_weight = in->var_weight;
  return LSDHIP_OK;
}
// ... 134 lines not shown
}
static void take_summary(lsdhip_tracker* t, const TrackSummary* S) {
  t->numEvaluations = S->numEvaluations;
  t->numWarpUpdates = S->numWarpUpdates;
  t->pointUsage = S->pointUsage; t->lastGoodCount = S->goodCount; t->lastBadCount = S->badCount; t->lastMeanRes = S->meanRes;
  t->affineEstimation_a = S->aff_a; t->affineEstimation_b = S->aff_b;
  t->affineEstimation_a_lastIt = S->aff_a_lastIt; t->affineEstimation_b_lastIt = S->aff_b_lastIt;
  t->lastResidual = S->lastResidual;
}
static bool tracking_was_good(const lsdhip_tracker* t, int level) {
  const lsdhip_ctx* c = t->ctx;
  return t->lastGoodCount / (c->wl[level] * c->hl[level]) > MIN_GOODPERALL_PIXEL &&
         t->lastGoodCount / (t->lastGoodCount + t->lastBadCount) > MIN_GOODPERGOODBAD_PIXEL;
}

static TrackScratch scratch_of(lsdhip_tracker* t) { return scratch_at(t, t->d_partials, 1, LSD_SPEC_MAX, LSD_SPEC_MAX); }
static void launch_step(lsdhip_tracker* t, const TrackJob& job, int grid, int parity, int first) {
  lsdhip_ctx* c = t->ctx;
  LSD_CTX_LOCK(c);
  TrackScratch sc = scratch_of(t);
  t->launchOrdinal++;
  t->spec.seq = t->jobTag ? ((t->jobTag << 12) | (t->launchOrdinal & 0xFFF)) : 0;
#ifdef LSD_DEVTOOLS
  t->spec.dbgLog = t->d_log;
#endif
#ifdef LSD_ORDER_CHECK
  t->spec.dbgCum = t->dbgCum;
  t->spec.dbgCounters = t->d_dbg;
  t->dbgCum += (unsigned long long)grid;
#endif
  hipLaunchKernelGGL((k_track_step<256, false>), dim3(grid), dim3(256), 0, c->stream, job, (const TrackJob*)nullptr, t->d_state, sc,
                     t->d_summary, parity, first, t->spec);
}
static int launch_steps(lsdhip_tracker* t, TrackJob& job, int steps, int* parity, int* first) {
  int grid = 1;
  for (int l = job.lastLevel; l <= job.topLevel; l++) if (job.lv[l].nblocks > grid) grid = job.lv[l].nblocks;
  t->spec.specGrid = 0;
  if (t->spec.specC > 1) {
    for (int l = job.lastLevel; l <= job.topLevel; l++) {
      const int g = job.lv[l].nblocks * (t->spec.trials[l] > 1 ? t->spec.trials[l] : 1);
      if (g > grid) grid = g;
    }
    t->spec.specGrid = grid;
  }
#ifdef LSD_DEVTOOLS
  const auto tl0 = std::chrono::steady_clock::now();
#endif
  for (int i = 0; i < steps; i++) {
    t->spec.last = (i + 1 == steps) ? 1 : 0;
    launch_step(t, job, grid, *parity, *first);
    lsdhip_host_mark(20);
    *first = 0;
    *parity ^= 1;
  }
#ifdef LSD_DEVTOOLS
  t->dbgEnqueued += steps;
  t->dbgLaunchNs += std::chrono::duration_cast<std::chrono::nanoseconds>(std::chrono::steady_clock::now() - tl0).count();
#endif
  HIPCHK(hipGetLastError());
  return LSDHIP_OK;
}

static int prof_collect(lsdhip_ctx* c);
struct EvalOut {
  int warped_size;
  float retval;
  float weightedError;
  float A[36], b[6], lsError;
  double num_constraints;
};

static void eval_out_of(const TrackSummary* S, EvalOut* eo) {
  const float* r = S->sums;
  int M = (int)r[RS_M];
  eo->warped_size = M;
  eo->retval = r[RS_SUMRES2] / r[RS_GOOD];
  eo->weightedError = r[RS_WERR] / ((M >> 2) << 2);
  size_t num_constraints = (size_t)6 * (size_t)(M >> 2);
  float n = (float)num_constraints;
  int k = RS_A0;
  for (int i = 0; i < 6; i++)
    for (int j = i; j < 6; j++, k++) {
      float v = (0.0f + r[k]) / n;
      eo->A[i * 6 + j] = v;
      eo->A[j * 6 + i] = v;
    }
  for (int i = 0; i < 6; i++) eo->b[i] = (0.0f - r[RS_B0 + i]) / n;
  eo->lsError = (0.0f + r[RS_ERR]) / n;
  eo->num_constraints = (double)num_constraints;
}

static int evaluate_pose(lsdhip_tracker* t, TrackJob& job, const lsdm::SE3fH& T, int level, EvalOut* eo) {
  lsdhip_ctx* c = t->ctx;
  LSD_CTX_LOCK(c);
  job.evalOnly = 1;
  job.lastLevel = level;
  job.topLevel = level;
  job.T0 = T;
  job.aff_a0 = t->affineEstimation_a; job.aff_b0 = t->affineEstimation_b;
  t->h_summary->done = 0;
  t->spec = TrackSpec{};
  t->jobTag = 0;
  if (int rcp = prof_collect(c)) return rcp;
  if (c->prof_on) HIPCHK(hipEventRecord(c->ev_a, c->stream));
  t->spec.last = 0;
  launch_step(t, job, job.lv[level].nblocks, 0, 1);
  if (c->prof_on) HIPCHK(hipEventRecord(c->ev_b, c->stream));
  launch_step(t, job, 1, 1, 0);
  HIPCHK(hipGetLastError());
  HIPCHK(hipStreamSynchronize(c->stream));
  const TrackSummary* S = t->h_summary;
  if (c->prof_on) {
    float ms = 0;
    HIPCHK(hipEventElapsedTime(&ms, c->ev_a, c->ev_b));
    c->prof_ms += ms;
    c->prof_launches++;
    c->prof_bytes += S->bytes;
  }
  t->numEvaluations++;
  t->pointUsage = S->pointUsage; t->lastGoodCount = S->goodCount; t->lastBadCount = S->badCount; t->lastMeanRes = S->meanRes;
  t->affineEstimation_a_lastIt = S->aff_a_lastIt; t->affineEstimation_b_lastIt = S->aff_b_lastIt;
  eval_out_of(S, eo);
  return LSDHIP_OK;
}

static void record_of(const TrackSummary* S, lsdhip_residual_record* out) {
  EvalOut ev;
// ... 87 lines not shown
    const unsigned want = *(volatile const unsigned*)&rec->check;
    if (chk == want) {
      if (spins > 0) {
        const long long ns = std::chrono::duration_cast<std::chrono::nanoseconds>(std::chrono::steady_clock::now() - t0).count();
        if (ns > t->sumLateMaxNs) t->sumLateMaxNs = ns;
        for (unsigned i = 1; i < LSD_SUMMARY_CHECK_WORDS; i++)
          if (first[i] != cur[i]) {
            t->sumLateWords++;
            if (t->sumLateFirstWord < 0 || (int)i < t->sumLateFirstWord) t->sumLateFirstWord = (int)i;
            if ((int)i > t->sumLateLastWord) t->sumLateLastWord = (int)i;
          }
      }
      std::atomic_thread_fence(std::memory_order_acquire);
      return LSDHIP_OK;
    }
    if (spins == 0) {
      t->sumLate++;
      t0 = std::chrono::steady_clock::now();
      memcpy(first, cur, sizeof(first));
    }
    if ((spins & 0xFFFFu) == 0xFFFFu && std::chrono::steady_clock::now() - t0 > std::chrono::seconds(2)) {
      lsd_set_error("tracking summary in pinned memory never became consistent (check %08x, sum %08x)", want, chk);
      return LSDHIP_E_STATE;
    }
    __builtin_ia32_pause();
  }
}
extern "C" int lsdhip_tracker_summary_stats(const lsdhip_tracker* t, long long out[6]) {
  if (!t || !out) return LSDHIP_E_ARG;
  out[0] = t->sumPolled; out[1] = t->sumLate; out[2] = t->sumLateMaxNs; out[3] = t->sumLateWords; out[4] = t->sumLateFirstWord; out[5] = t->sumLateLastWord;
  return LSDHIP_OK;
}

static int track_device(lsdhip_tracker* t, TrackJob& job, int topLevel, const lsdm::SE3fH& T0, lsdm::SE3fH* Tout) {
  lsdhip_ctx* c = t->ctx;
  job.evalOnly = 0;
  job.topLevel = topLevel;
  job.T0 = T0;
  job.aff_a0 = 1.0f; job.aff_b0 = 0.0f;
  t->spec.specC = t->specC;
  t->spec.specGrid = 0;
  t->maskSet ^= 1;
  t->spec.wasGoodSide = t->d_maskSide + (size_t)t->maskSet * t->maskStride * (LSD_SPEC_MAX - 1);
  t->spec.maskStride = (unsigned)t->maskStride;
  t->spec.copyMask = c->pipeline ? 0 : 1;
  if (c->pipeline && t->maskMergeSeq[t->maskSet] != 0) {
    if (t->maskMergeSeq[t->maskSet] < 0) { if (int rcf = lsd_flush_merges(c)) return rcf; }
    if (t->maskMergeSeq[t->maskSet] > c->mSeq && lsd_m_record(c) < 0) return LSDHIP_E_HIP;
    if (int rcw = lsd_t_wait_m(c, t->maskMergeSeq[t->maskSet])) return rcw;
    t->maskMergeSeq[t->maskSet] = 0;
  }
  for (int l = 0; l < LSD_LEVELS; l++) t->spec.trials[l] = 1;
  if (t->specC > 1) {
    for (int l = job.lastLevel; l <= topLevel; l++) {
      TrackLevel& L = job.lv[l];
      const long long work = L.npts >= 0 ? L.npts : (long long)L.w * L.h;
      int trials, cap = t->specCaps[l];
      if (t->specLevel[l] > 0) trials = t->specLevel[l];
      else if (!t->specAuto) trials = t->specC;
      else trials = work <= LSD_SPEC_SMALL_PX ? LSD_SPEC_TRIALS_SMALL : (work <= LSD_SPEC_MID_PX ? LSD_SPEC_TRIALS_MID : 1);
      if (trials > t->specC) trials = t->specC;
      if (cap <= 0 && trials > 1 && (t->specAuto ? work > LSD_SPEC_CAP_ABOVE_PX : l == job.lastLevel)) cap = t->specCap > 0 ? t->specCap : ((t->grid_cap / 2 + 7) & ~7);
      t->spec.trials[l] = trials;
      if (trials > 1 && cap > 0 && L.nblocks > cap && L.tilePx == 0) {
        L.nblocks = cap;
        L.singlePass = (long long)L.nblocks * t->block >= work ? 1 : 0;
      }
    }
  }
  t->h_summary->done = 0;
  const TrackSummary* S = t->h_summary;
  const long long myEpoch = ++c->enqEpoch;
  int budget = 12;
  if (t->recent[0] > 0) {
    budget = 0;
    for (int i = 0; i < 4; i++) if (t->recent[i] > budget) budget = t->recent[i];
    budget += t->budgetExtra;
  }
  if (t->budgetFixed > 0) budget = t->budgetFixed;
  const bool sample = c->prof_on && ((c->prof_tick++ & 7) == 0);
#ifdef LSD_DEVTOOLS
  t->dbgJobs++;
#endif
  t->jobTag = (t->jobTag % 0x7FFFF) + 1;
  t->launchOrdinal = 0;
  t->h_summary->seq = 0;
  t->h_summary->exhausted = 0;
  int guard = 0;
  int parity = 0, first = 1;
  if (int rc = prof_collect(c)) return rc;
  lsdhip_host_mark(2);
  while (true) {
    if (sample) HIPCHK(hipEventRecord(c->ev_a, c->stream));
    int rc = LSDHIP_OK;
    rc = launch_steps(t, job, budget, &parity, &first);
    if (rc) return rc;
    if (sample) { HIPCHK(hipEventRecord(c->ev_b, c->stream)); c->prof_pending = true; }
    lsdhip_host_mark(3);
    if (guard == 0 && t->enqueueHook && job.trackFrameSemantics) t->enqueueHook(t->enqueueHookUser);
    lsdhip_host_mark(4);
#ifdef LSD_DEVTOOLS
    const auto tw0 = std::chrono::steady_clock::now();
    struct WaitClock { lsdhip_tracker* t; std::chrono::steady_clock::time_point t0; ~WaitClock() { t->dbgWaitNs += std::chrono::duration_cast<std::chrono::nanoseconds>(std::chrono::steady_clock::now() - t0).count(); } } waitClock_{t, tw0};
#endif
    c->mtx.unlock();
    struct Relock { std::recursive_mutex& m; ~Relock() { m.lock(); } };
    {
    Relock relock_{c->mtx};
    if (t->spinWait) {
      volatile const int* done = &S->done;
      volatile const int* exhausted = &S->exhausted;
      const int lastSeq = t->spec.seq;
      const auto tStart = std::chrono::steady_clock::now();
      unsigned spins = 0;
      while (*done != t->jobTag) {
        if (*exhausted == lastSeq) break;
        if ((++spins & 0xFFFFFu) == 0) {
          hipError_t q = hipStreamQuery(c->stream);
          if (q == hipSuccess) break;
          if (q != hipErrorNotReady) { lsd_set_error("hipStreamQuery failed: %s", hipGetErrorString(q)); return LSDHIP_E_HIP; }
          if (std::chrono::steady_clock::now() - tStart > std::chrono::seconds(5)) { HIPCHK(hipStreamSynchronize(c->stream)); break; }
        }
        __builtin_ia32_pause();
      }
      std::atomic_thread_fence(std::memory_order_acquire);
    } else {
      HIPCHK(hipStreamSynchronize(c->stream));
    }
    }
    lsdhip_host_mark(5);
    if (*(volatile const int*)&S->done == t->jobTag) break;
#ifdef LSD_DEVTOOLS
    t->dbgMisses++;
#endif
    HIPCHK(hipStreamSynchronize(c->stream));
#ifdef LSD_DEVTOOLS
    {
      static const bool dumpL0 = getenv("LSDHIP_DUMP_L0") != nullptr;
      if (dumpL0 && guard == 0 && t->budgetFixed == 1) {
        const TrackScratch sc = scratch_of(t);
        const size_t rows = (size_t)t->max_blocks;
        const int nb = job.lv[topLevel].nblocks;
        t->dumpL0.assign((size_t)nb * (RS_COLS + 4 + 96) + sizeof(TrackState) / 4, 0u);
        unsigned* d = t->dumpL0.data();
        HIPCHK(hipMemcpy(d, sc.sums + (size_t)(1 * LSD_SPEC_MAX + 0) * RS_COLS * rows, (size_t)nb * RS_COLS * 4, hipMemcpyDeviceToHost));
        HIPCHK(hipMemcpy(d + (size_t)nb * RS_COLS, sc.topkey + (size_t)(1 * LSD_SPEC_MAX + 0) * rows, (size_t)nb * 16, hipMemcpyDeviceToHost));
        HIPCHK(hipMemcpy(d + (size_t)nb * (RS_COLS + 4), sc.topval + (size_t)(1 * LSD_SPEC_MAX + 0) * rows * 96, (size_t)nb * 96 * 4, hipMemcpyDeviceToHost));
        HIPCHK(hipMemcpy(d + (size_t)nb * (RS_COLS + 4 + 96), t->d_state + 1, sizeof(TrackState), hipMemcpyDeviceToHost));
      }
    }
#endif
    if (*(volatile const int*)&S->done == t->jobTag) break;
    if (int rc2 = prof_collect(c)) return rc2;
    if (t->jobKf && t->jobKf->depthVersion != t->jobKfVersion && guard < 8) {
      t->jobKfVersion = t->jobKf->depthVersion;
      t->h_summary->done = 0;
      parity = 0; first = 1;
      budget = 12;
      ++guard;
      continue;
    }
    budget = t->budgetFixed > 0 ? t->budgetFixed : 6;
    if (++guard > 200) { lsd_set_error("tracking job did not terminate"); return LSDHIP_E_STATE; }
  }
  if (int rcs = summary_wait_consistent(t, t->jobTag)) return rcs;
  if (sample) {
    c->prof_bytes += S->bytes;
    c->prof_launches += S->numLaunches;
  }
  if (myEpoch > c->doneEpoch) c->doneEpoch = myEpoch;
#ifdef LSD_DEVTOOLS
  {
    static const bool keepLog = getenv("LSDHIP_LAUNCH_LOG") != nullptr;
    if (keepLog) {
      HIPCHK(hipStreamSynchronize(c->stream));
      const int n = t->launchOrdinal < 4095 ? t->launchOrdinal + 1 : 4096;
      t->lastLog.assign((size_t)n * 16, 0);
      HIPCHK(hipMemcpy(t->lastLog.data(), t->d_log, (size_t)n * 64, hipMemcpyDeviceToHost));
      HIPCHK(hipMemset(t->d_log, 0, (size_t)n * 64));
    }
  }
#endif
  t->numLaunches = S->numLaunches;
  t->recent[3] = t->recent[2]; t->recent[2] = t->recent[1]; t->recent[1] = t->recent[0]; t->recent[0] = t->numLaunches;
  for (int l = 0; l < LSD_LEVELS; l++) t->levelEvaluations[l] = S->levelEvals[l];
  take_summary(t, S);
  *Tout = pose_of(S);
  return S->diverged ? LSDHIP_DIVERGED : LSDHIP_OK;
}

static void fill_result(lsdhip_tracker* t, const lsdm::SE3dH& T, lsdhip_track_result* out) {
  lsdm::se3d_to7(T, out->frameToReference);
  out->pointUsage = t->pointUsage; out->lastGoodCount = t->lastGoodCount; out->lastBadCount = t->lastBadCount;
  out->lastMeanRes = t->lastMeanRes; out->lastResidual = t->lastResidual;
  out->affineEstimation_a = t->affineEstimation_a; out->affineEstimation_b = t->affineEstimation_b;
  out->diverged = t->diverged; out->trackingWasGood = t->trackingWasGood;
  out->numEvaluations = t->numEvaluations; out->numWarpUpdates = t->numWarpUpdates;
}
static lsdm::SE3dH identity_d() { lsdm::SE3dH I; I.q = {1, 0, 0, 0}; I.t[0] = I.t[1] = I.t[2] = 0; return I; }
static int finish_diverged(lsdhip_tracker* t, lsdhip_track_result* out) {
  t->diverged = true;
  t->trackingWasGood = false;
  fill_result(t, identity_d(), out);
  return LSDHIP_DIVERGED;
}

static int fill_trackframe_job(lsdhip_tracker* t, TrackJob& job, BatchShape shape, lsdhip_frame* kf, lsdhip_frame* frame) {
  fill_job_common(t, job);
  for (int lvl = LSD_TRACK_MIN_LEVEL; lvl < LSD_TRACK_MAX_LEVEL; lvl++)
    if (int rcl = fill_level(t, job, shape, lvl, kf, frame, nullptr, nullptr, -1)) return rcl;
  job.lv[LSD_TRACK_MIN_LEVEL].writeMask = 1;
  int rc = lsd_frame_ensure_wasgood(frame);
  if (rc) return rc;
  job.wasGood = frame->d_wasGood;
  job.lastLevel = LSD_TRACK_MIN_LEVEL;
// ... 96 lines not shown
  {
    unsigned long long pv = 0;
    for (int i = 0; i < 7; i++) { unsigned long long u; memcpy(&u, &init[i], 8); pv = pv * 1000003ull + u; }
    lsd_trace_val(c, 22, frame->id, pv);
    lsd_trace_val(c, 23, frame->id, (unsigned long long)kf->id);
  }
#endif
  lsdm::SE3fH referenceToFrame = lsdm::se3f_from_d(lsdm::se3d_inverse(lsdm::se3d_from7(init)));

  if (t->hostLM) {
    float last_residual = 0;
    rc = LSDHIP_OK;
    for (int lvl = LSD_TRACK_MAX_LEVEL - 1; lvl >= LSD_TRACK_MIN_LEVEL && rc == LSDHIP_OK; lvl--)
      rc = lm_level_host(t, job, lvl, referenceToFrame, &last_residual);
    t->lastResidual = last_residual;
    if (rc == LSDHIP_DIVERGED) return finish_diverged(t, out);
    if (rc) return rc;
    TrackSummary S = *t->h_summary;
    S.diverged = 0;
    S.q[0] = referenceToFrame.q.w; S.q[1] = referenceToFrame.q.x; S.q[2] = referenceToFrame.q.y; S.q[3] = referenceToFrame.q.z;
    S.t[0] = referenceToFrame.t[0]; S.t[1] = referenceToFrame.t[1]; S.t[2] = referenceToFrame.t[2];
    S.lastResidual = last_residual; S.numEvaluations = t->numEvaluations; S.numWarpUpdates = t->numWarpUpdates;
    S.pointUsage = t->pointUsage; S.goodCount = t->lastGoodCount; S.badCount = t->lastBadCount; S.meanRes = t->lastMeanRes;
    S.aff_a = t->affineEstimation_a; S.aff_b = t->affineEstimation_b;
    S.aff_a_lastIt = t->affineEstimation_a_lastIt; S.aff_b_lastIt = t->affineEstimation_b_lastIt;
    return finish_trackframe(t, &S, kf, frame, out);
  }
  t->jobKf = kf;
  t->jobKfVersion = kf->depthVersion;
#ifdef LSD_DEVTOOLS
  const lsdm::SE3fH referenceToFrame0 = referenceToFrame;
  lsd_trace_val(c, 26, frame->id, t->dbgCum / 400ull);
#endif
  rc = track_device(t, job, LSD_TRACK_MAX_LEVEL - 1, referenceToFrame, &referenceToFrame);
  if (rc != LSDHIP_OK && rc != LSDHIP_DIVERGED) { t->jobKf = nullptr; return rc; }
#ifdef LSD_DEVTOOLS
  static const bool replay = getenv("LSDHIP_TRACK_REPLAY") != nullptr;
  if (replay && c->pipeline) {
    unsigned long long pv = 0;
    for (int i = 0; i < 4; i++) { unsigned u; memcpy(&u, &t->h_summary->q[i], 4); pv = pv * 1000003ull + u; }
    for (int i = 0; i < 3; i++) { unsigned u; memcpy(&u, &t->h_summary->t[i], 4); pv = pv * 1000003ull + u; }
    lsd_trace_val(c, 24, frame->id, pv);
    lsd_trace_val(c, 25, frame->id, (unsigned long long)t->h_summary->numEvaluations * 1000 + t->h_summary->lastCand);
    HIPCHK(hipStreamSynchronize(c->mstream));
    HIPCHK(hipStreamSynchronize(c->stream));
    c->mDoneSeq = c->mSeq;
    const std::vector<unsigned> dump1 = t->dumpL0;
    if (traceInputs) trace_inputs(100);
    lsd_trace_val(c, 27, frame->id, t->dbgCum / 400ull);
    referenceToFrame = referenceToFrame0;
    rc = track_device(t, job, LSD_TRACK_MAX_LEVEL - 1, referenceToFrame, &referenceToFrame);
    if (rc != LSDHIP_OK && rc != LSDHIP_DIVERGED) { t->jobKf = nullptr; return rc; }
    HIPCHK(hipStreamSynchronize(c->stream));
    if (!dump1.empty() && dump1.size() == t->dumpL0.size()) {
      const int nb = job.lv[LSD_TRACK_MAX_LEVEL - 1].nblocks;
      int shown = 0;
      for (size_t i = 0; i < dump1.size(); i++)
        if (dump1[i] != t->dumpL0[i] && shown++ < 12) {
          const size_t a = (size_t)nb * RS_COLS, b = a + (size_t)nb * 4, cst = b + (size_t)nb * 96;
          float f1, f2; memcpy(&f1, &dump1[i], 4); memcpy(&f2, &t->dumpL0[i], 4);
          if (i < a) fprintf(stderr, "L0DIFF frame %d: sums tile %zu column %zu: run %.9g (%08x) replay %.9g (%08x)\n", frame->id, i / RS_COLS, i % RS_COLS, f1, dump1[i], f2, t->dumpL0[i]);
          else if (i < b) fprintf(stderr, "L0DIFF frame %d: topkey tile %zu [%zu]: run %d replay %d\n", frame->id, (i - a) / 4, (i - a) % 4, (int)dump1[i], (int)t->dumpL0[i]);
          else if (i < cst) fprintf(stderr, "L0DIFF frame %d: topval tile %zu slot %zu entry %zu: run %.9g replay %.9g\n", frame->id, (i - b) / 96, ((i - b) % 96) / 32, (i - b) % 32, f1, f2);
          else fprintf(stderr, "L0DIFF frame %d: state word %zu: run %08x (%.9g) replay %08x (%.9g)\n", frame->id, i - cst, dump1[i], f1, t->dumpL0[i], f2);
        }
      if (shown) fprintf(stderr, "L0DIFF frame %d: %d words differ after the first launch\n", frame->id, shown);
    }
// ... 480 lines not shown
```

### lsd_slam_amd/driver.py

```python
import ctypes as C
import os

import numpy as np

from . import capi

_HERE = os.path.dirname(os.path.abspath(__file__))
DRIVER_PATH = os.path.join(_HERE, "liblsdhip_driver.so")
_lib = None


class LoopStats(C.Structure):
    _fields_ = [("seconds_track", C.c_double), ("seconds_map", C.c_double), ("seconds_keyframe", C.c_double), ("frames", C.c_longlong),
                ("updates", C.c_longlong), ("keyframes", C.c_longlong), ("evaluations", C.c_longlong), ("tracked_good", C.c_longlong),
                ("level_evaluations", C.c_longlong * 5), ("track_launches", C.c_longlong), ("dropped", C.c_longlong)]


EXPORTED_SYMBOLS = ["lsdloop_create", "lsdloop_destroy", "lsdloop_run", "lsdloop_get_stats", "lsdloop_reset_stats",
                    "lsdloop_copy_keyframe_planes", "lsdloop_set_keyframe_ring", "lsdloop_keyframes_exported", "lsdloop_ctx",
                    "lsdloop_last_error", "lsdloop_keep_keyframes", "lsdloop_keyframe_log", "lsdloop_set_live_queue", "lsdloop_set_pipeline", "lsdloop_set_speculation", "lsdloop_observe_time", "lsdloop_comm_unique_id", "lsdloop_comm_init", "lsdloop_comm_destroy",
                    "lsdloop_gather_keyframes", "lsdband_create", "lsdband_destroy", "lsdband_window_rows", "lsdband_layout", "lsdband_load",
                    "lsdband_get", "lsdband_comm_init", "lsdband_run", "lsdband_synchronize", "lsdband_halo_bytes_per_pass", "lsdband_set_packed_exchange", "lsdband_set_overlap", "lsdband_tile_runs", "lsdband_plan", "lsdband_ipc_init", "lsdband_ipc_connect", "lsdband_ipc_failed", "lsdloop_gather_counts", "lsdloop_ipc_init", "lsdloop_ipc_connect", "lsdloop_ipc_result", "lsdloop_observe_work",
                    "lsdloopbatch_create", "lsdloopbatch_destroy", "lsdloopbatch_run", "lsdloopbatch_get_stats", "lsdloopbatch_ctx", "lsdloopbatch_set_keyframe_phases", "lsdloopbatch_set_pipeline", "lsdloopbatch_set_coarse_min_jobs", "lsdloopbatch_dropped",
                    "lsdloopbatch_keep_keyframes", "lsdloopbatch_keyframe_log", "lsdloopbatch_last_result", "lsdloopbatch_download_map",
                    "lsdloopbatch_set_cloud_sinks", "lsdloopbatch_cloud", "lsdloopbatch_cloud_pose", "lsdloopbatch_keyframe_handle"]


def lib():
    global _lib
    if _lib is None:
        capi.lib()
        if not os.path.exists(DRIVER_PATH):
            raise RuntimeError("liblsdhip_driver.so is missing (%s): run __graft_entry__.build()" % DRIVER_PATH)
        L = C.CDLL(DRIVER_PATH)
        vp, i = C.c_void_p, C.c_int
        L.lsdloop_create.restype = i
        L.lsdloop_create.argtypes = [i, i, i, vp, vp, i, vp, i, C.POINTER(vp)]
        L.lsdloop_destroy.restype = None
        L.lsdloop_destroy.argtypes = [vp]
        L.lsdloop_run.restype = i
        L.lsdloop_run.argtypes = [vp, vp, i, i, vp]
        L.lsdloop_get_stats.restype = i
        L.lsdloop_get_stats.argtypes = [vp, C.POINTER(LoopStats)]
        L.lsdloop_reset_stats.restype = i
        L.lsdloop_reset_stats.argtypes = [vp]
        L.lsdloop_copy_keyframe_planes.restype = i
        L.lsdloop_copy_keyframe_planes.argtypes = [vp, vp, vp]
        L.lsdloop_set_keyframe_ring.restype = i
        L.lsdloop_set_keyframe_ring.argtypes = [vp, vp, i]
        L.lsdloop_keyframes_exported.restype = C.c_longlong
        L.lsdloop_keyframes_exported.argtypes = [vp]
        L.lsdloop_keep_keyframes.restype = i
        L.lsdloop_keep_keyframes.argtypes = [vp, i]
        L.lsdloop_keyframe_log.restype = i
        L.lsdloop_keyframe_log.argtypes = [vp, vp, vp, i]
        L.lsdloop_set_live_queue.restype = i
        L.lsdloop_set_live_queue.argtypes = [vp, i]
        L.lsdloop_set_pipeline.restype = i
        L.lsdloop_set_pipeline.argtypes = [vp, i]
        L.lsdloop_set_speculation.restype = i
        L.lsdloop_set_speculation.argtypes = [vp, i, i]
        L.lsdloop_observe_time.restype = i
        L.lsdloop_observe_time.argtypes = [vp, vp, vp]
        L.lsdloop_observe_work.restype = i
        L.lsdloop_observe_work.argtypes = [vp, vp]
        L.lsdloop_comm_unique_id.restype = i
        L.lsdloop_comm_unique_id.argtypes = [vp]
        for name, args in (("lsdband_create", [i, i, i, i, i, i, C.POINTER(vp)]), ("lsdband_window_rows", [vp]), ("lsdband_layout", [vp, i, vp]),
                           ("lsdband_load", [vp, i, vp, vp]), ("lsdband_get", [vp, i, vp]), ("lsdband_comm_init", [vp, vp, i, i, vp]),
                           ("lsdband_run", [vp, i]), ("lsdband_synchronize", [vp]), ("lsdband_set_packed_exchange", [vp, i]), ("lsdband_set_overlap", [vp, i]), ("lsdband_tile_runs", [i, i, i, vp, i]), ("lsdband_plan", [i, i, vp, vp, vp, i]),
                           ("lsdband_ipc_init", [vp, i, i, vp, vp]), ("lsdband_ipc_connect", [vp, vp]), ("lsdband_ipc_failed", [vp])):
            getattr(L, name).restype = i
            getattr(L, name).argtypes = args
        L.lsdband_destroy.restype = None
        L.lsdband_destroy.argtypes = [vp]
        L.lsdband_halo_bytes_per_pass.restype = C.c_longlong
        L.lsdband_halo_bytes_per_pass.argtypes = [vp]
        L.lsdloop_comm_init.restype = i
        L.lsdloop_comm_init.argtypes = [vp, vp, i, i]
        L.lsdloop_comm_destroy.restype = i
        L.lsdloop_comm_destroy.argtypes = [vp]
        L.lsdloop_gather_keyframes.restype = i
        L.lsdloop_gather_keyframes.argtypes = [vp, i, i, vp, C.c_longlong]
        for name, args in (("lsdloop_gather_counts", [vp, vp, i]), ("lsdloop_ipc_init", [vp, i, i, i, vp]), ("lsdloop_ipc_connect", [vp, vp]),
                           ("lsdloop_ipc_result", [vp, vp, vp])):
            getattr(L, name).restype = i
            getattr(L, name).argtypes = args
        L.lsdloop_ctx.restype = vp
        L.lsdloop_ctx.argtypes = [vp]
        L.lsdloopbatch_create.restype = i
        L.lsdloopbatch_create.argtypes = [i, i, i, vp, i, vp, i, vp, i, C.POINTER(vp)]
        L.lsdloopbatch_destroy.restype = None
        L.lsdloopbatch_destroy.argtypes = [vp]
        L.lsdloopbatch_run.restype = i
# ... 125 lines not shown

    def set_keyframe_phases(self, phases):
        a = (C.c_int * self.S)(*[int(p) for p in phases])
        _check(self.L.lsdloopbatch_set_keyframe_phases(self.h_, a))


class DriverLoop:

    def __init__(self, w, h, K, first_image_ptr, depth0, kf_every=10, images_on_device=True, device=0):
        self.L = lib()
        K4 = np.ascontiguousarray(K, dtype=np.float32)
        d0 = np.ascontiguousarray(depth0, dtype=np.float32)
        h_ = C.c_void_p()
        _check(self.L.lsdloop_create(device, w, h, K4.ctypes.data, C.c_void_p(first_image_ptr), int(images_on_device),
                                     d0.ctypes.data, kf_every, C.byref(h_)))
        self.h_ = h_
        self.w, self.h = w, h

    def close(self):
        if getattr(self, "h_", None):
            self.L.lsdloop_destroy(self.h_)
            self.h_ = None

    def __del__(self):
        self.close()

    def run(self, image_ptrs, stop_at_keyframe=False, want_poses=False):
        n = len(image_ptrs)
        arr = (C.c_void_p * n)(*image_ptrs)
        poses = np.zeros((n, 7), np.float64) if want_poses else None
        done = _check(self.L.lsdloop_run(self.h_, arr, n, int(stop_at_keyframe), poses.ctypes.data if want_poses else None))
        return done, (poses[:done] if want_poses else None)

    def stats(self):
        s = LoopStats()
        _check(self.L.lsdloop_get_stats(self.h_, C.byref(s)))
        return s

    def reset_stats(self):
        _check(self.L.lsdloop_reset_stats(self.h_))

    def copy_keyframe_planes(self, idepth_ptr, var_ptr):
        _check(self.L.lsdloop_copy_keyframe_planes(self.h_, C.c_void_p(idepth_ptr), C.c_void_p(var_ptr)))

    def set_keyframe_ring(self, ring_ptr, slots):
        _check(self.L.lsdloop_set_keyframe_ring(self.h_, C.c_void_p(ring_ptr) if ring_ptr else None, slots))

    def gather_counts(self, world):
        out = (C.c_int * world)()
        n = _check(self.L.lsdloop_gather_counts(self.h_, out, world))
        return list(out)[:n]

    def ipc_init(self, rank, world, root=0):
        out = (C.c_ubyte * 64)()
        _check(self.L.lsdloop_ipc_init(self.h_, rank, world, root, out))
        self._ipc_world = world
        return bytes(out)

    def ipc_connect(self, root_handle):
        buf = (C.c_ubyte * 64).from_buffer_copy(root_handle)
        _check(self.L.lsdloop_ipc_connect(self.h_, buf))

    def ipc_result(self):
        counts = (C.c_int * self._ipc_world)()
        ptr = C.c_void_p()
        fail = self.L.lsdloop_ipc_result(self.h_, counts, C.byref(ptr))
# ... 55 lines not shown
```

### lsd_slam_amd/driver/slam_loop.cpp

```cpp
#include <chrono>
#include <cstdlib>
#include <cstring>
#include <dlfcn.h>
#include <string>

#include "../../include/lsd_slam_hip.hpp"
#include "../../include/lsdhip_driver.h"

using namespace lsd_slam_hip;

static thread_local std::string g_err;
typedef void* NcclComm;

struct lsdloop {
  std::unique_ptr<SlamLoop> loop;
  std::shared_ptr<Context> ctx;
  lsdloop_stats st{};
  double wall = 0;
  double gpu0[3] = {0, 0, 0};
  long long calls0[3] = {0, 0, 0};
  float* ring = nullptr;
  int ring_slots = 0;
  long long ring_count = 0;
  NcclComm comm = nullptr;
// ... 226 lines not shown
  try {
    const auto& log = l->loop->sequence(s).keyframeLog;
    for (int i = 0; i < (int)log.size() && i < max; i++) {
      if (scales_out) scales_out[i] = log[i]->thisToParent_raw().s;
      if (points_out) points_out[i] = log[i]->stats().numPoints;
    }
    return (int)log.size();
  } catch (const Error& e) { g_err = e.what(); return e.status < 0 ? e.status : LSDHIP_E_STATE; }
}
extern "C" int lsdloopbatch_last_result(lsdloopbatch* l, int s, lsdhip_track_result* out) {
  if (!l || !out || s < 0 || s >= l->loop->size()) return LSDHIP_E_ARG;
  *out = l->loop->sequence(s).last;
  return LSDHIP_OK;
}
extern "C" int lsdloopbatch_download_map(lsdloopbatch* l, int s, lsdhip_hypothesis* out) {
  if (!l || !out || s < 0 || s >= l->loop->size()) return LSDHIP_E_ARG;
  try {
    const std::vector<lsdhip_hypothesis> m = l->loop->sequence(s).map.currentDepthMap();
    std::memcpy(out, m.data(), m.size() * sizeof(lsdhip_hypothesis));
    return LSDHIP_OK;
  } catch (const Error& e) { g_err = e.what(); return e.status < 0 ? e.status : LSDHIP_E_STATE; }
}
extern "C" int lsdloopbatch_set_keyframe_phases(lsdloopbatch* l, const int* phase) {
  if (!l || !phase) return LSDHIP_E_ARG;
  try {
    l->loop->setKeyframePhases(std::vector<int>(phase, phase + l->loop->size()));
    return LSDHIP_OK;
  } catch (const Error& e) {
    g_err = e.what();
    return e.status < 0 ? e.status : LSDHIP_E_STATE;
  }
}

extern "C" int lsdloop_run(lsdloop* l, const uint8_t* const* images, int n, int stop_at_keyframe, double* out7) {
  if (!l || !images || n < 0) return LSDHIP_E_ARG;
  try {
    int done = 0;
    long updSeen = l->loop->numUpdates;
    static const bool prefetch = !std::getenv("LSDHIP_NO_PREFETCH");
    const double t0 = now_s();
    for (int i = 0; i < n; i++) {
      SlamLoop& L = *l->loop;
      const long ev0 = L.evaluations;
      const long la0 = L.launches;
      const long good0 = L.numTrackedGood;
      const long drop0 = L.numDropped;
      long lev0[5];
      for (int k = 0; k < 5; k++) lev0[k] = L.levelEvaluations[k];
      SE3 est = L.step(images[i], [](double) {}, (prefetch && i + 1 < n) ? images[i + 1] : nullptr);
      l->st.frames++;
      l->st.updates += L.numUpdates - updSeen;
      updSeen = L.numUpdates;
      l->st.evaluations += L.evaluations - ev0;
      l->st.track_launches += L.launches - la0;
      l->st.tracked_good += L.numTrackedGood - good0;
      l->st.dropped += L.numDropped - drop0;
      for (int k = 0; k < 5; k++) l->st.level_evaluations[k] += L.levelEvaluations[k] - lev0[k];
      if (L.newKeyframe) l->st.keyframes++;
      if (out7) est.to7(out7 + 7 * (size_t)i);
      done++;
      if (stop_at_keyframe && L.newKeyframe) break;
    }
    l->loop->flushDeferredMapping();
    {
      const long upd = l->loop->numUpdates - updSeen;
      l->st.updates += upd;
    }
    l->ctx->synchronize();
    l->wall += now_s() - t0;
    return done;
  } catch (const Error& e) {
    g_err = e.what();
    return e.status > 0 ? -100 - e.status : e.status;
  } catch (const std::exception& e) {
    g_err = e.what();
    return LSDHIP_E_STATE;
  }
}
extern "C" int lsdloop_get_stats(lsdloop* l, lsdloop_stats* out) {
  if (!l || !out) return LSDHIP_E_ARG;
  try {
    double ms[3];
    long long calls[3];
    l->loop->map.gpuTimes(ms, calls);
    auto scaled = [&](int k, long n) {
      const long long sampled = calls[k] - l->calls0[k];
      if (sampled > 0) return (ms[k] - l->gpu0[k]) / (double)sampled * (double)n * 1e-3;
      return calls[k] > 0 ? ms[k] / (double)calls[k] * (double)n * 1e-3 : 0.0;
    };
    l->st.seconds_map = scaled(0, l->st.updates);
    l->st.seconds_keyframe = scaled(1, l->st.keyframes) + scaled(2, l->st.keyframes);
    l->st.seconds_track = l->loop->pipelined() ? l->wall : l->wall - l->st.seconds_map - l->st.seconds_keyframe;
    *out = l->st;
    return LSDHIP_OK;
  } catch (const Error& e) { g_err = e.what(); return e.status; }
}
extern "C" int lsdloop_reset_stats(lsdloop* l) {
  if (!l) return LSDHIP_E_ARG;
  try {
    l->loop->map.gpuTimes(l->gpu0, l->calls0);
    l->st = lsdloop_stats{};
    l->wall = 0;
    return LSDHIP_OK;
  } catch (const Error& e) { g_err = e.what(); return e.status; }
}
extern "C" int lsdloop_copy_keyframe_planes(lsdloop* l, float* idepth_dev, float* var_dev) {
  if (!l) return LSDHIP_E_ARG;
  try { l->loop->map.copyPlanesToDevice(idepth_dev, var_dev); return LSDHIP_OK; }
  catch (const Error& e) { g_err = e.what(); return e.status; }
}
// ... 610 lines not shown
```

Measured before the change: 5351.

## Chain next frame's tracking onto the persistent tracker kernel as a successor job

Adds a 'succession' mechanism: while a frame is being tracked, the prefetched next frame is attached as a successor job, so the device kernel can start tracking it as soon as the current track converges. The next frame starts from a pose derived from the current result, with tags used to tell the main job apart from the successor. The aim is to remove per-frame host round trips and launch gaps between consecutive tracks. The cost is considerable state-management complexity: successors must be abandoned on keyframe changes, depth updates or divergence, and extra kernel branches add some register and control overhead.

After: 5228. -2.3%, worse.

```diff
diff --git a/include/lsd_slam_hip.hpp b/include/lsd_slam_hip.hpp
--- a/include/lsd_slam_hip.hpp
+++ b/include/lsd_slam_hip.hpp
@@ -367,6 +367,15 @@
   int numEvaluations = 0, numWarpUpdates = 0;
   int levelEvaluations[LSDHIP_PYRAMID_LEVELS] = {0, 0, 0, 0, 0};
   int numLaunches = 0;
+  void offerSuccessor(Frame* next) { check(lsdhip_tracker_offer_successor(h_, next ? next->handle() : nullptr), "lsdhip_tracker_offer_successor"); }
+  void cancelSuccessor() { check(lsdhip_tracker_cancel_successor(h_), "lsdhip_tracker_cancel_successor"); }
+  void setSuccession(bool on) { check(lsdhip_tracker_set_succession(h_, on ? 1 : 0), "lsdhip_tracker_set_succession"); }
+  struct SuccessionStats { long long attached, adopted, abandoned; bool on; };
+  SuccessionStats successionStats() const {
+    long long o[4];
+    check(lsdhip_tracker_succession_stats(h_, o), "lsdhip_tracker_succession_stats");
+    return {o[0], o[1], o[2], o[3] != 0};
+  }
   void setSpeculation(int trials, int finestLevelWorkgroups = 0) { check(lsdhip_tracker_set_speculation(h_, trials, finestLevelWorkgroups), "lsdhip_tracker_set_speculation"); }
   void setBatchCoarseMinJobs(int minJobs) { check(lsdhip_tracker_set_batch_coarse_min_jobs(h_, minJobs), "lsdhip_tracker_set_batch_coarse_min_jobs"); }
 
@@ -559,8 +568,11 @@
       if (!pendingNext_) return;
       prefetched_ = makeFrame(frameId_ + 1, pendingNext_, true);
       prefetchedSrc_ = pendingNext_;
+      const bool changesKeyframe = kfEvery_ > 0 && sinceKF_ + 1 >= kfEvery_;
+      if (!pendingKF_ && !changesKeyframe) tracker.offerSuccessor(prefetched_.get());
     });
   }
+  ~SlamLoop() { try { tracker.cancelSuccessor(); } catch (...) {} }
   SlamLoop(const SlamLoop&) = delete;
   SlamLoop& operator=(const SlamLoop&) = delete;
   void setPipelined(bool on) {
@@ -587,8 +599,12 @@
     lsdhip_host_mark(0);
     frameId_++;
     std::shared_ptr<Frame> frame;
-    if (prefetched_ && prefetchedSrc_ == image) frame = std::move(prefetched_);
-    else frame = makeFrame(frameId_, image);
+    if (prefetched_ && prefetchedSrc_ == image) {
+      frame = std::move(prefetched_);
+    } else {
+      if (prefetched_) tracker.cancelSuccessor();
+      frame = makeFrame(frameId_, image);
+    }
     prefetched_.reset();
     pendingNext_ = nextImage;
     if (!pipelined_ && keyframe->depthHasBeenUpdatedFlag()) {
diff --git a/include/lsdhip.h b/include/lsdhip.h
--- a/include/lsdhip.h
+++ b/include/lsdhip.h
@@ -134,6 +134,10 @@
                                    int level, int repeats, double* ms_per_launch, double* bytes_per_launch);
 typedef void (*lsdhip_enqueue_hook)(void* user);
 int lsdhip_tracker_set_enqueue_hook(lsdhip_tracker* t, lsdhip_enqueue_hook fn, void* user);
+int lsdhip_tracker_offer_successor(lsdhip_tracker* t, lsdhip_frame* next);
+int lsdhip_tracker_cancel_successor(lsdhip_tracker* t);
+int lsdhip_tracker_set_succession(lsdhip_tracker* t, int on);
+int lsdhip_tracker_succession_stats(const lsdhip_tracker* t, long long out[4]);
 int lsdhip_tracker_track(lsdhip_tracker* t, lsdhip_frame* keyframe, lsdhip_frame* frame,
                          const double frameToReference_initialEstimate[7], lsdhip_track_result* out);
 int lsdhip_tracker_track_batch(lsdhip_tracker* t, int n, lsdhip_frame** keyframes, lsdhip_frame** frames,
diff --git a/include/lsdhip_driver.h b/include/lsdhip_driver.h
--- a/include/lsdhip_driver.h
+++ b/include/lsdhip_driver.h
@@ -22,6 +22,10 @@
                    const float* gt_depth0_host, int kf_every, lsdloop** out);
 void lsdloop_destroy(lsdloop* l);
 int lsdloop_run(lsdloop* l, const uint8_t* const* images, int n, int stop_at_keyframe, double* frameToKeyframe_out);
+int lsdloop_run_frames(lsdloop* l, const uint8_t* const* images, const uint8_t* const* next_images, int n, double* frameToKeyframe_out,
+                       long long* per_frame_out);
+int lsdloop_set_succession(lsdloop* l, int on);
+int lsdloop_succession_stats(lsdloop* l, long long out[4]);
 int lsdloop_get_stats(lsdloop* l, lsdloop_stats* out);
 int lsdloop_reset_stats(lsdloop* l);
 int lsdloop_copy_keyframe_planes(lsdloop* l, float* idepth_dev, float* idepthVar_dev);
diff --git a/lsd_slam_amd/capi.py b/lsd_slam_amd/capi.py
--- a/lsd_slam_amd/capi.py
+++ b/lsd_slam_amd/capi.py
@@ -133,6 +133,10 @@
         "lsdhip_tracker_summary_stats": (i, [vp, vp]),
         "lsdhip_tracker_step_stats": (i, [vp, vp]),
         "lsdhip_tracker_set_enqueue_hook": (i, [vp, vp, vp]),
+        "lsdhip_tracker_offer_successor": (i, [vp, vp]),
+        "lsdhip_tracker_cancel_successor": (i, [vp]),
+        "lsdhip_tracker_set_succession": (i, [vp, i]),
+        "lsdhip_tracker_succession_stats": (i, [vp, vp]),
         "lsdhip_tracker_track": (i, [vp, vp, vp, vp, C.POINTER(TrackResult)]),
         "lsdhip_tracker_track_batch": (i, [vp, i, pvp, pvp, vp, C.POINTER(TrackResult)]),
         "lsdhip_tracker_eval_throughput": (i, [vp, i, pvp, pvp, vp, i, i, C.POINTER(C.c_double), C.POINTER(C.c_double)]),
diff --git a/lsd_slam_amd/csrc/lsdhip_internal.hpp b/lsd_slam_amd/csrc/lsdhip_internal.hpp
--- a/lsd_slam_amd/csrc/lsdhip_internal.hpp
+++ b/lsd_slam_amd/csrc/lsdhip_internal.hpp
@@ -66,6 +66,17 @@
   int writeMask;
 };
 
+struct TrackSummary;
+struct TrackSucc {
+  const float4* fr_grad[LSD_LEVELS];
+  const float* kf_idepth[LSD_LEVELS];
+  const float* kf_idepthVar[LSD_LEVELS];
+  uint8_t* wasGood;
+  uint8_t* wasGoodSide;
+  TrackSummary* out;
+  int tag;
+  int has;
+};
 struct TrackJob {
   TrackLevel lv[LSD_LEVELS];
   uint8_t* wasGood;
@@ -78,6 +89,7 @@
   float aff_a0, aff_b0;
   int evalOnly;
   int trackFrameSemantics;
+  TrackSucc succ;
 };
 struct TrackSpec {
   int specC;
@@ -117,6 +129,8 @@
   int ncand;
   int lastCand;
   int numLaunches;
+  int tag;
+  lsdm::SE3fH succT0;
 };
 
 struct TrackSummary {
@@ -129,6 +143,8 @@
   int levelEvals[LSD_LEVELS];
   int numLaunches;
   int lastCand;
+  float succT0[7];
+  int succPad_;
   int seq;
   int exhausted;
   unsigned check;
@@ -331,6 +347,30 @@
   long long dbgJobs = 0, dbgEnqueued = 0, dbgMisses = 0, dbgWaitNs = 0, dbgLaunchNs = 0;
   TrackSummary* h_summary = nullptr;
   TrackSummary* d_summary = nullptr;
+  TrackSummary* h_summary2 = nullptr;
+  TrackSummary* d_summary2 = nullptr;
+  int sumRec = 0;
+  bool succession = false;
+  lsdhip_frame* succOffer = nullptr;
+  struct Successor {
+    bool attached = false;
+    lsdhip_frame* frame = nullptr;
+    const lsdhip_frame* kf = nullptr;
+    unsigned kfVersion = 0;
+    TrackJob job;
+    int trials[LSD_LEVELS];
+    int specC = 0;
+    int tag = 0, rec = 0, maskSet = 0;
+    long long epoch = 0;
+    int firstLaunch = 0;
+  } succ;
+  int chainLaunches = 0;
+  int chainParity = 0;
+  int prevNeeded = 0;
+  float prevSuccT0[7] = {};
+  int tagReserve = 0;
+  int budgetExtraSucc = 3;
+  long long succAttached = 0, succAdopted = 0, succAbandoned = 0;
   unsigned long long* d_trace = nullptr;
   int batch_capacity = 0;
   TrackJob* d_bjobs = nullptr;
diff --git a/lsd_slam_amd/csrc/pose_math.hpp b/lsd_slam_amd/csrc/pose_math.hpp
--- a/lsd_slam_amd/csrc/pose_math.hpp
+++ b/lsd_slam_amd/csrc/pose_math.hpp
@@ -78,6 +78,7 @@
   q_rotate<Quatf, float>(r.q, nt, r.t);
   return r;
 }
+LSDM_HD SE3fH successor_pose(const SE3fH& T) { return se3f_from_d(se3d_inverse(se3d_from_f(se3f_inverse(T)))); }
 LSDM_HD SE3fH se3f_mul(const SE3fH& a, const SE3fH& b) {
   SE3fH r = a;
   float rt[3];
diff --git a/lsd_slam_amd/csrc/track_device.hpp b/lsd_slam_amd/csrc/track_device.hpp
--- a/lsd_slam_amd/csrc/track_device.hpp
+++ b/lsd_slam_amd/csrc/track_device.hpp
@@ -354,6 +354,9 @@
   for (int l = 0; l < LSD_LEVELS; l++) SUM_PUT_IA(levelEvals, l, s.levelEvals[l]);
   SUM_PUT_I(numLaunches, s.numLaunches);
   SUM_PUT_I(lastCand, s.lastCand);
+  SUM_PUT_FA(succT0, 0, s.succT0.q.w); SUM_PUT_FA(succT0, 1, s.succT0.q.x); SUM_PUT_FA(succT0, 2, s.succT0.q.y); SUM_PUT_FA(succT0, 3, s.succT0.q.z);
+  SUM_PUT_FA(succT0, 4, s.succT0.t[0]); SUM_PUT_FA(succT0, 5, s.succT0.t[1]); SUM_PUT_FA(succT0, 6, s.succT0.t[2]);
+  SUM_PUT_I(succPad_, 0);
 #undef SUM_PUT_I
 #undef SUM_PUT_F
 #undef SUM_PUT_IA
@@ -370,8 +373,9 @@
 struct LmPar {
   float lambdaInitial, stepSizeMin, convergenceEps, minWarped, lambdaSuccessFac, lambdaFailFac;
   int maxIts, w, h, writeMask, evalOnly, useAffine, tfSemantics, lastLevel, trials;
+  int succ;
 };
-__device__ __forceinline__ void stage_lm_par(const TrackJob& job, int level, LmPar& p, const int trials = 1) {
+__device__ __forceinline__ void stage_lm_par(const TrackJob& job, int level, LmPar& p, const int trials = 1, const int succ = 0) {
   const TrackLevel& L = job.lv[level];
   LmPar v;
   v.lambdaInitial = L.lambdaInitial; v.stepSizeMin = L.stepSizeMin; v.convergenceEps = L.convergenceEps; v.minWarped = L.minWarped;
@@ -379,6 +383,7 @@
   v.maxIts = L.maxIts; v.w = L.w; v.h = L.h; v.writeMask = L.writeMask; v.evalOnly = job.evalOnly; v.useAffine = job.useAffine;
   v.tfSemantics = job.trackFrameSemantics; v.lastLevel = job.lastLevel;
   v.trials = trials;
+  v.succ = succ;
   p = v;
 }
 
@@ -520,6 +525,7 @@
   if (!tfSemantics) S.last_residual = lastErr;
   if (S.level == L.lastLevel) {
     S.done = 1;
+    if (L.succ) S.succT0 = lsdm::successor_pose(T);
     if (out && lane == 0) write_summary(S, tot, out, doneWord);
   } else {
     S.level = S.level - 1;
@@ -557,10 +563,13 @@
   acc[RS_ERR] = __builtin_fmaf(resw, o.res, acc[RS_ERR]);
 }
 
-__device__ __forceinline__ void make_ctx_dev(const TrackJob& jobr, const TrackState& S, int level, EvalCtx& a) {
+__device__ __forceinline__ void make_ctx_dev(const TrackJob& jobr, const TrackState& S, int level, EvalCtx& a, const bool onSucc = false) {
   const TrackJob* job = &jobr;
   const TrackLevel& L = job->lv[level];
-  a.kf_idepth = (gfloat*)L.kf_idepth; a.kf_idepthVar = (gfloat*)L.kf_idepthVar; a.kf_image = (gfloat*)L.kf_image; a.fr_grad = (gfloat*)L.fr_grad;
+  a.kf_idepth = (gfloat*)(onSucc ? job->succ.kf_idepth[level] : L.kf_idepth);
+  a.kf_idepthVar = (gfloat*)(onSucc ? job->succ.kf_idepthVar[level] : L.kf_idepthVar);
+  a.kf_image = (gfloat*)L.kf_image;
+  a.fr_grad = (gfloat*)(onSucc ? (const float*)job->succ.fr_grad[level] : (const float*)L.fr_grad);
   a.pts_pos = (gfloat*)L.pts_pos; a.pts_colvar = (gfloat*)L.pts_colvar; a.npts = L.npts; a.w = L.w; a.h = L.h;
   a.fx = L.fx; a.fy = L.fy; a.cx = L.cx; a.cy = L.cy; a.fxi = L.fxi; a.fyi = L.fyi; a.cxi = L.cxi; a.cyi = L.cyi;
 #pragma unroll
diff --git a/lsd_slam_amd/csrc/tracker.hip b/lsd_slam_amd/csrc/tracker.hip
--- a/lsd_slam_amd/csrc/tracker.hip
+++ b/lsd_slam_amd/csrc/tracker.hip
@@ -22,10 +22,11 @@
 #endif
 
 enum { TS_FUSED = 0, TS_LM = 1, TS_EVAL = 2 };
-__device__ __forceinline__ void track_state_begin(TrackState& S, const TrackJob& job, const int tid) {
+__device__ __forceinline__ void track_state_begin(TrackState& S, const TrackJob& job, const int tid, const lsdm::SE3fH& T0, const int tag) {
   if (tid == 0) {
-    S.T = job.T0;
-    set_eval_pose(S, job.T0);
+    S.T = T0;
+    set_eval_pose(S, T0);
+    S.tag = tag; S.succT0 = T0;
     S.aff_a = job.aff_a0; S.aff_b = job.aff_b0; S.aff_a_lastIt = job.aff_a0; S.aff_b_lastIt = job.aff_b0;
     S.lastErr = 0; S.LM_lambda = 0; S.last_residual = 0;
     S.level = job.topLevel; S.iteration = 0; S.incTry = 0; S.phase = 0; S.pending = 0;
@@ -125,10 +126,14 @@
   }
 #endif
   PHASE_MARK(0);
-  if (!BATCH && MODE == TS_FUSED && !first && !leader && st2[parity].done) return;
-  if (!BATCH && MODE == TS_FUSED && leader && tid == 0 && spec.seq != 0) out->seq = spec.seq;
+  const int mainTag = (MODE == TS_FUSED && spec.seq != 0) ? (BATCH ? spec.seq : (spec.seq >> 12)) : 1;
+  constexpr bool SUCC = !BATCH && MODE == TS_FUSED;
+  if (SUCC && !first && !leader) {
+    const TrackState* sp = st2 + parity;
+    if (sp->done && !(job.succ.has && sp->tag == mainTag && !sp->diverged)) return;
+  }
   if (first) {
-    track_state_begin(S, job, tid);
+    track_state_begin(S, job, tid, job.T0, mainTag);
   } else {
     copy_words<sizeof(TrackState) / 4>(&S, st2 + parity, tid, BLOCK);
     if (SPEC_LM && cmax > 1 && tid < 32 * TRIALS_MAX) (&s_rec[0][0])[tid] = sc.recs[(size_t)parity * cmax * 32 + (tid < 32 * cmax ? tid : 0)];
@@ -139,13 +144,30 @@
   const int lvlIn_ = S.level, numLaunchesIn_ = S.numLaunches, pendingIn_ = S.pending, ncandIn_ = S.ncand;
   int pcLog_ = -1;
 #endif
-  if (S.done) {
+  bool onSucc = false;
+  if (SUCC && !first && job.succ.has) {
+    const int sTag = S.tag;
+    if (sTag == job.succ.tag) {
+      onSucc = true;
+    } else if (sTag == mainTag && S.done && !S.diverged) {
+      const lsdm::SE3fH T0s = S.succT0;
+      __syncthreads();
+      track_state_begin(S, job, tid, T0s, job.succ.tag);
+      __syncthreads();
+      onSucc = true;
+    }
+  }
+  if (S.done || (SUCC && !first && !onSucc && S.tag != mainTag)) {
     LAUNCH_LOG(1, pendingIn_, ncandIn_, -1);
     if (MODE != TS_EVAL && leader) { copy_words<sizeof(TrackState) / 4>(next, &S, tid, BLOCK); }
     return;
   }
+  if (SUCC && leader && tid == 0 && spec.seq != 0) out->seq = spec.seq;
   const int lvlPending = S.level;
-  const int doneWord = (MODE == TS_FUSED && spec.seq != 0) ? (BATCH ? spec.seq : (spec.seq >> 12)) : 1;
+  const int doneWord = onSucc ? job.succ.tag : mainTag;
+  TrackSummary* const outJob = onSucc ? job.succ.out : out;
+  uint8_t* const jobWasGood = onSucc ? job.succ.wasGood : job.wasGood;
+  uint8_t* const sideMasks = onSucc ? job.succ.wasGoodSide : spec.wasGoodSide;
   if (MODE == TS_FUSED) {
     const int nbl = job.lv[lvlPending].nblocks;
     const int tr = (spec.specC > 1 && spec.trials[lvlPending] > 1) ? spec.trials[lvlPending] : 1;
@@ -276,7 +298,7 @@
           if (lane < 6 && c >= 0) key = second ? (r == 0 ? keysB[0] : (r == 1 ? keysB[1] : keysB[2])) : (r == 0 ? keysA[0] : (r == 1 ? keysA[1] : keysA[2]));
           if (key >= 0) {
             EvalCtx a;
-            make_ctx_dev(job, S, level, a);
+            make_ctx_dev(job, S, level, a, onSucc);
             if (c > 0) {
               const float* rec = s_rec[c];
 #pragma unroll
@@ -368,7 +390,7 @@
         else tail_two(ca, cb, std::integral_constant<int, 5>());
       }
     };
-    if (tid == SUMW * 64 - 1) stage_lm_par(job, level, s_par, (spec.specC > 1 && spec.trials[level] > 1) ? spec.trials[level] : 1);
+    if (tid == SUMW * 64 - 1) stage_lm_par(job, level, s_par, (spec.specC > 1 && spec.trials[level] > 1) ? spec.trials[level] : 1, SUCC && job.succ.has && !onSucc);
     if (wave < SUMW) {
       const int t = tid;
       const int slot_ = t / (RS_COLS / 4);
@@ -513,9 +535,9 @@
         PHASE_MARK(3);
 #ifdef LSD_PHASE_TRACE
         if (trOn_ && tid == 0) { tr_[19] = (unsigned long long)ncandPending; tr_[7] = (unsigned long long)pc; }
-        lm_wave<SPEC_LM>(s_par, S, s, sh.tot, tid, leader ? out : nullptr, trOn_ ? tr_ : nullptr, pc, cand, doneWord);
+        lm_wave<SPEC_LM>(s_par, S, s, sh.tot, tid, leader ? outJob : nullptr, trOn_ ? tr_ : nullptr, pc, cand, doneWord);
 #else
-        lm_wave<SPEC_LM>(s_par, S, s, sh.tot, tid, leader ? out : nullptr, nullptr, pc, cand, doneWord);
+        lm_wave<SPEC_LM>(s_par, S, s, sh.tot, tid, leader ? outJob : nullptr, nullptr, pc, cand, doneWord);
 #endif
       }
     }
@@ -523,14 +545,14 @@
     PHASE_MARK(4);
     if (S.done) {
       if (!BATCH && MODE == TS_FUSED && S.lastCand > 0 && spec.copyMask != 0 && job.lv[level].writeMask && cand == 0 && bx < nb) {
-        const uint8_t* side = spec.wasGoodSide + (size_t)(S.lastCand - 1) * spec.maskStride;
+        const uint8_t* side = sideMasks + (size_t)(S.lastCand - 1) * spec.maskStride;
         EvalCtx a;
-        make_ctx_dev(job, S, level, a);
+        make_ctx_dev(job, S, level, a, onSucc);
         const int work = a.npts >= 0 ? a.npts : a.w * a.h;
         for (int i = bx * BLOCK + tid; i < work; i += nb * BLOCK) {
           float px, py, pz, I_ref, var;
           int maskIdx;
-          if (fetch_point(a, i, px, py, pz, I_ref, var, maskIdx) && maskIdx >= 0) job.wasGood[maskIdx] = side[maskIdx];
+          if (fetch_point(a, i, px, py, pz, I_ref, var, maskIdx) && maskIdx >= 0) jobWasGood[maskIdx] = side[maskIdx];
         }
       }
       if (leader) copy_words<sizeof(TrackState) / 4>(next, &S, tid, BLOCK);
@@ -564,7 +586,7 @@
   topval_out += (size_t)cand * max_rows * 96;
   const int tile = xcd_tile(bx, nb);
   EvalCtx a;
-  make_ctx_dev(job, S, level, a);
+  make_ctx_dev(job, S, level, a, onSucc);
   if (BATCH && MODE == TS_EVAL && cand > 0) {
     const float* rec = sc.recs + ((size_t)parity * cmax + cand) * 32;
 #pragma unroll
@@ -572,7 +594,7 @@
 #pragma unroll
     for (int i = 0; i < 3; i++) a.t[i] = rec[22 + i];
   }
-  gbyte* wasGood = (gbyte*)(job.lv[level].writeMask ? (cand == 0 ? job.wasGood : spec.wasGoodSide + (size_t)(cand - 1) * spec.maskStride) : nullptr);
+  gbyte* wasGood = (gbyte*)(job.lv[level].writeMask ? (cand == 0 ? jobWasGood : sideMasks + (size_t)(cand - 1) * spec.maskStride) : nullptr);
   const int work = a.npts >= 0 ? a.npts : a.w * a.h;
   float acc[RS_END];
 #pragma unroll
@@ -783,7 +805,7 @@
   }
   if (MODE == TS_FUSED && leader) copy_words<sizeof(TrackState) / 4>(next, &S, tid, BLOCK);
  
-  if (MODE == TS_FUSED && leader && tid == 0 && spec.last != 0) out->exhausted = spec.seq;
+  if (MODE == TS_FUSED && leader && tid == 0 && spec.last != 0 && !onSucc) out->exhausted = spec.seq;
   LAUNCH_LOG(3, pendingIn_, ncandIn_, S.lastCand);
   PHASE_MARK(6);
 #ifdef LSD_PHASE_TRACE
@@ -849,7 +871,7 @@
   __shared__ v4f s_tex[LSD_SOLO_MAX_PX];
   __shared__ float s_var[LSD_SOLO_LDS_PTS], s_img[LSD_SOLO_LDS_PTS];
   const int tid = threadIdx.x, wave = tid >> 6, lane = tid & 63;
-  track_state_begin(S, job, tid);
+  track_state_begin(S, job, tid, job.T0, 0);
   __syncthreads();
   int listLevel = -1, total = 0;
   EvalCtx a;
@@ -1218,13 +1240,17 @@
   HIPCHK(hipMalloc((void**)&t->d_trace, (1 + 4096 * LSD_TRACE_WORDS) * 8));
   HIPCHK(hipMemsetAsync(t->d_trace, 0, (1 + 4096 * LSD_TRACE_WORDS) * 8, c->stream));
 #endif
-  HIPCHK(hipHostMalloc((void**)&t->h_summary, sizeof(TrackSummary), hipHostMallocMapped));
-  HIPCHK(hipHostGetDevicePointer((void**)&t->d_summary, t->h_summary, 0));
-  memset(t->h_summary, 0, sizeof(TrackSummary));
+  HIPCHK(hipHostMalloc((void**)&t->h_summary2, 2 * sizeof(TrackSummary), hipHostMallocMapped));
+  HIPCHK(hipHostGetDevicePointer((void**)&t->d_summary2, t->h_summary2, 0));
+  memset(t->h_summary2, 0, 2 * sizeof(TrackSummary));
+  t->h_summary = t->h_summary2;
+  t->d_summary = t->d_summary2;
   const char* env = getenv("LSDHIP_HOST_LM");
   t->hostLM = env && env[0] == '1';
   if (const char* e = getenv("LSDHIP_SPIN")) t->spinWait = e[0] != '0';
   if (const char* e = getenv("LSDHIP_BUDGET_EXTRA")) { t->budgetExtra = atoi(e); if (t->budgetExtra < 1) t->budgetExtra = 1; }
+  if (const char* e = getenv("LSDHIP_BUDGET_EXTRA_SUCC")) { t->budgetExtraSucc = atoi(e); if (t->budgetExtraSucc < 1) t->budgetExtraSucc = 1; }
+  if (const char* e = getenv("LSDHIP_SUCCESSION")) t->succession = e[0] != '0';
   if (const char* e = getenv("LSDHIP_BUDGET_FIXED")) { t->budgetFixed = atoi(e); if (t->budgetFixed < 1) t->budgetFixed = 0; }
   *out = t;
   return LSDHIP_OK;
@@ -1285,7 +1311,7 @@
 #ifdef LSD_DEVTOOLS
   (void)hipFree(t->d_log);
 #endif
-  (void)hipHostFree(t->h_summary);
+  (void)hipHostFree(t->h_summary2);
   if (t->d_pts) (void)hipFree(t->d_pts);
   delete t;
 }
@@ -1486,7 +1512,7 @@
   hipLaunchKernelGGL((k_track_step<256, false>), dim3(grid), dim3(256), 0, c->stream, job, (const TrackJob*)nullptr, t->d_state, sc,
                      t->d_summary, parity, first, t->spec);
 }
-static int launch_steps(lsdhip_tracker* t, TrackJob& job, int steps, int* parity, int* first) {
+static int launch_steps(lsdhip_tracker* t, TrackJob& job, int steps, int* parity, int* first, bool endsBudget = true) {
   int grid = 1;
   for (int l = job.lastLevel; l <= job.topLevel; l++) if (job.lv[l].nblocks > grid) grid = job.lv[l].nblocks;
   t->spec.specGrid = 0;
@@ -1501,9 +1527,10 @@
   const auto tl0 = std::chrono::steady_clock::now();
 #endif
   for (int i = 0; i < steps; i++) {
-    t->spec.last = (i + 1 == steps) ? 1 : 0;
+    t->spec.last = (endsBudget && i + 1 == steps) ? 1 : 0;
     launch_step(t, job, grid, *parity, *first);
     lsdhip_host_mark(20);
+    t->chainLaunches = *first ? 1 : t->chainLaunches + 1;
     *first = 0;
     *parity ^= 1;
   }
@@ -1544,9 +1571,11 @@
   eo->num_constraints = (double)num_constraints;
 }
 
+static int cancel_successor(lsdhip_tracker* t);
 static int evaluate_pose(lsdhip_tracker* t, TrackJob& job, const lsdm::SE3fH& T, int level, EvalOut* eo) {
   lsdhip_ctx* c = t->ctx;
   LSD_CTX_LOCK(c);
+  if (int rcs = cancel_successor(t)) return rcs;
   job.evalOnly = 1;
   job.lastLevel = level;
   job.topLevel = level;
@@ -1700,7 +1729,156 @@
   return LSDHIP_OK;
 }
 
-static int track_device(lsdhip_tracker* t, TrackJob& job, int topLevel, const lsdm::SE3fH& T0, lsdm::SE3fH* Tout) {
+static void apply_speculation(const lsdhip_tracker* t, TrackJob& job, int topLevel, int trialsOut[LSD_LEVELS]) {
+  for (int l = 0; l < LSD_LEVELS; l++) trialsOut[l] = 1;
+  if (t->specC <= 1) return;
+  for (int l = job.lastLevel; l <= topLevel; l++) {
+    TrackLevel& L = job.lv[l];
+    const long long work = L.npts >= 0 ? L.npts : (long long)L.w * L.h;
+    int trials, cap = t->specCaps[l];
+    if (t->specLevel[l] > 0) trials = t->specLevel[l];
+    else if (!t->specAuto) trials = t->specC;
+    else trials = work <= LSD_SPEC_SMALL_PX ? LSD_SPEC_TRIALS_SMALL : (work <= LSD_SPEC_MID_PX ? LSD_SPEC_TRIALS_MID : 1);
+    if (trials > t->specC) trials = t->specC;
+    if (cap <= 0 && trials > 1 && (t->specAuto ? work > LSD_SPEC_CAP_ABOVE_PX : l == job.lastLevel)) cap = t->specCap > 0 ? t->specCap : ((t->grid_cap / 2 + 7) & ~7);
+    trialsOut[l] = trials;
+    if (trials > 1 && cap > 0 && L.nblocks > cap && L.tilePx == 0) {
+      L.nblocks = cap;
+      L.singlePass = (long long)L.nblocks * t->block >= work ? 1 : 0;
+    }
+  }
+}
+static uint8_t* mask_side_set(const lsdhip_tracker* t, int set) { return t->d_maskSide + (size_t)set * t->maskStride * (LSD_SPEC_MAX - 1); }
+static int wait_mask_merge(lsdhip_tracker* t, int set) {
+  lsdhip_ctx* c = t->ctx;
+  if (!c->pipeline || t->maskMergeSeq[set] == 0) return LSDHIP_OK;
+  if (t->maskMergeSeq[set] < 0) { if (int rcf = lsd_flush_merges(c)) return rcf; }
+  if (t->maskMergeSeq[set] > c->mSeq && lsd_m_record(c) < 0) return LSDHIP_E_HIP;
+  if (int rcw = lsd_t_wait_m(c, t->maskMergeSeq[set])) return rcw;
+  t->maskMergeSeq[set] = 0;
+  return LSDHIP_OK;
+}
+static void use_summary_record(lsdhip_tracker* t, int rec) {
+  t->sumRec = rec;
+  t->h_summary = t->h_summary2 + rec;
+  t->d_summary = t->d_summary2 + rec;
+}
+static int abandon_successor(lsdhip_tracker* t) {
+  lsdhip_tracker::Successor& s = t->succ;
+  if (!s.attached) return LSDHIP_OK;
+  s.attached = false;
+  t->succAbandoned++;
+  lsdhip_ctx* c = t->ctx;
+  if (s.frame && s.frame->d_wasGood) HIPCHK(hipMemsetAsync(s.frame->d_wasGood, 0xFF, (size_t)c->wl[1] * c->hl[1], c->stream));
+  return LSDHIP_OK;
+}
+static int cancel_successor(lsdhip_tracker* t) {
+  if (!t->succ.attached) return LSDHIP_OK;
+  if (int rc = abandon_successor(t)) return rc;
+  HIPCHK(hipStreamSynchronize(t->ctx->stream));
+  return LSDHIP_OK;
+}
+extern "C" int lsdhip_tracker_cancel_successor(lsdhip_tracker* t) {
+  if (!t) return LSDHIP_E_ARG;
+  LSD_CTX_LOCK(t->ctx);
+  HIPCHK(hipSetDevice(t->ctx->device));
+  t->succOffer = nullptr;
+  return cancel_successor(t);
+}
+extern "C" int lsdhip_tracker_offer_successor(lsdhip_tracker* t, lsdhip_frame* next) {
+  if (!t) return LSDHIP_E_ARG;
+  t->succOffer = next;
+  return LSDHIP_OK;
+}
+extern "C" int lsdhip_tracker_set_succession(lsdhip_tracker* t, int on) {
+  if (!t) return LSDHIP_E_ARG;
+  LSD_CTX_LOCK(t->ctx);
+  t->succession = on != 0;
+  return LSDHIP_OK;
+}
+extern "C" int lsdhip_tracker_succession_stats(const lsdhip_tracker* t, long long out[4]) {
+  if (!t || !out) return LSDHIP_E_ARG;
+  out[0] = t->succAttached; out[1] = t->succAdopted; out[2] = t->succAbandoned; out[3] = t->succession ? 1 : 0;
+  return LSDHIP_OK;
+}
+static int fill_trackframe_job(lsdhip_tracker* t, TrackJob& job, BatchShape shape, lsdhip_frame* kf, lsdhip_frame* frame);
+static bool attach_successor(lsdhip_tracker* t, TrackJob& job, int topLevel) {
+  lsdhip_ctx* c = t->ctx;
+  lsdhip_frame* nf = t->succOffer;
+  t->succOffer = nullptr;
+  lsdhip_frame* kf = const_cast<lsdhip_frame*>(t->jobKf);
+  if (!t->succession || !nf || !kf || !c->pipeline || !t->spinWait || !job.trackFrameSemantics || job.evalOnly || t->succ.attached) return false;
+  lsdhip_tracker::Successor& s = t->succ;
+  if (fill_trackframe_job(t, s.job, BatchShape{}, kf, nf) != LSDHIP_OK) return false;
+  const bool pend = kf->depthPending;
+  if (pend)
+    for (int l = LSD_TRACK_MIN_LEVEL; l < LSD_TRACK_MAX_LEVEL; l++) {
+      s.job.lv[l].kf_idepth = kf->d_idepthW[l]; s.job.lv[l].kf_idepthVar = kf->d_idepthVarW[l]; s.job.lv[l].kf_refBlk = kf->d_refBlkW[l];
+    }
+  s.job.evalOnly = 0;
+  s.job.topLevel = topLevel;
+  s.job.aff_a0 = 1.0f; s.job.aff_b0 = 0.0f;
+  apply_speculation(t, s.job, topLevel, s.trials);
+  if (memcmp(s.trials, t->spec.trials, sizeof(s.trials)) != 0) return false;
+  {
+    TrackJob same = s.job;
+    for (int l = 0; l < LSD_LEVELS; l++) {
+      same.lv[l].fr_grad = job.lv[l].fr_grad; same.lv[l].kf_idepth = job.lv[l].kf_idepth; same.lv[l].kf_idepthVar = job.lv[l].kf_idepthVar;
+      same.lv[l].kf_refBlk = job.lv[l].kf_refBlk;
+    }
+    same.wasGood = job.wasGood;
+    same.T0 = job.T0;
+    if (memcmp(&same, &job, sizeof(TrackJob)) != 0) return false;
+  }
+  const int set = t->maskSet ^ 1;
+  if (wait_mask_merge(t, set) != LSDHIP_OK) return false;
+  long long need = nf->readySeq > kf->readySeq ? nf->readySeq : kf->readySeq;
+  const long long dseq = pend ? kf->depthPendingSeq : kf->depthSeq;
+  if (dseq > need) need = dseq;
+  if (lsd_t_wait_m(c, need) != LSDHIP_OK) return false;
+  s.frame = nf;
+  s.kf = kf;
+  s.kfVersion = kf->depthVersion + (pend ? 1u : 0u);
+  s.specC = t->specC;
+  s.tag = (t->jobTag % 0x7FFFF) + 1;
+  s.rec = t->sumRec ^ 1;
+  s.maskSet = set;
+  s.epoch = ++c->enqEpoch;
+  s.firstLaunch = t->chainLaunches + 1;
+  TrackSummary* r = t->h_summary2 + s.rec;
+  r->done = 0; r->seq = 0; r->exhausted = 0;
+  std::atomic_thread_fence(std::memory_order_release);
+  TrackSucc& k = job.succ;
+  for (int l = 0; l < LSD_LEVELS; l++) { k.fr_grad[l] = s.job.lv[l].fr_grad; k.kf_idepth[l] = s.job.lv[l].kf_idepth; k.kf_idepthVar[l] = s.job.lv[l].kf_idepthVar; }
+  k.wasGood = s.job.wasGood;
+  k.wasGoodSide = mask_side_set(t, set);
+  k.out = t->d_summary2 + s.rec;
+  k.tag = s.tag;
+  k.has = 1;
+  s.attached = true;
+  t->tagReserve = s.tag;
+  t->succAttached++;
+  return true;
+}
+static int adopt_successor(lsdhip_tracker* t, const TrackJob& job, const lsdm::SE3fH& T0, const lsdhip_frame* frame) {
+  lsdhip_tracker::Successor& s = t->succ;
+  if (!s.attached) return 0;
+  const lsdhip_ctx* c = t->ctx;
+  bool ok = t->succession && c->pipeline && t->spinWait && frame && s.frame == frame && s.kf == t->jobKf && t->jobKf->depthVersion == s.kfVersion &&
+            s.specC == t->specC && memcmp(s.trials, t->spec.trials, sizeof(s.trials)) == 0;
+  if (ok) {
+    TrackJob want = s.job;
+    want.T0 = job.T0;
+    ok = memcmp(&want, &job, sizeof(TrackJob)) == 0;
+  }
+  const float T7[7] = {T0.q.w, T0.q.x, T0.q.y, T0.q.z, T0.t[0], T0.t[1], T0.t[2]};
+  ok = ok && memcmp(T7, t->prevSuccT0, sizeof(T7)) == 0;
+  const int begun = t->prevNeeded + 1 > s.firstLaunch ? t->prevNeeded + 1 : s.firstLaunch;
+  ok = ok && t->prevNeeded > 0 && t->chainLaunches >= begun;
+  return ok ? t->chainLaunches - begun + 1 : 0;
+}
+
+static int track_device(lsdhip_tracker* t, TrackJob& job, int topLevel, const lsdm::SE3fH& T0, lsdm::SE3fH* Tout, lsdhip_frame* frame = nullptr) {
   lsdhip_ctx* c = t->ctx;
   job.evalOnly = 0;
   job.topLevel = topLevel;
@@ -1708,64 +1886,81 @@
   job.aff_a0 = 1.0f; job.aff_b0 = 0.0f;
   t->spec.specC = t->specC;
   t->spec.specGrid = 0;
-  t->maskSet ^= 1;
-  t->spec.wasGoodSide = t->d_maskSide + (size_t)t->maskSet * t->maskStride * (LSD_SPEC_MAX - 1);
   t->spec.maskStride = (unsigned)t->maskStride;
   t->spec.copyMask = c->pipeline ? 0 : 1;
-  if (c->pipeline && t->maskMergeSeq[t->maskSet] != 0) {
-    if (t->maskMergeSeq[t->maskSet] < 0) { if (int rcf = lsd_flush_merges(c)) return rcf; }
-    if (t->maskMergeSeq[t->maskSet] > c->mSeq && lsd_m_record(c) < 0) return LSDHIP_E_HIP;
-    if (int rcw = lsd_t_wait_m(c, t->maskMergeSeq[t->maskSet])) return rcw;
-    t->maskMergeSeq[t->maskSet] = 0;
-  }
-  for (int l = 0; l < LSD_LEVELS; l++) t->spec.trials[l] = 1;
-  if (t->specC > 1) {
-    for (int l = job.lastLevel; l <= topLevel; l++) {
-      TrackLevel& L = job.lv[l];
-      const long long work = L.npts >= 0 ? L.npts : (long long)L.w * L.h;
-      int trials, cap = t->specCaps[l];
-      if (t->specLevel[l] > 0) trials = t->specLevel[l];
-      else if (!t->specAuto) trials = t->specC;
-      else trials = work <= LSD_SPEC_SMALL_PX ? LSD_SPEC_TRIALS_SMALL : (work <= LSD_SPEC_MID_PX ? LSD_SPEC_TRIALS_MID : 1);
-      if (trials > t->specC) trials = t->specC;
-      if (cap <= 0 && trials > 1 && (t->specAuto ? work > LSD_SPEC_CAP_ABOVE_PX : l == job.lastLevel)) cap = t->specCap > 0 ? t->specCap : ((t->grid_cap / 2 + 7) & ~7);
-      t->spec.trials[l] = trials;
-      if (trials > 1 && cap > 0 && L.nblocks > cap && L.tilePx == 0) {
-        L.nblocks = cap;
-        L.singlePass = (long long)L.nblocks * t->block >= work ? 1 : 0;
-      }
-    }
-  }
-  t->h_summary->done = 0;
+  apply_speculation(t, job, topLevel, t->spec.trials);
+  t->succOffer = nullptr;
+  const int had = adopt_successor(t, job, T0, frame);
+  long long myEpoch;
+  int parity = 0, first = 1;
+  if (had > 0) {
+    const lsdhip_tracker::Successor& s = t->succ;
+    t->maskSet = s.maskSet;
+    use_summary_record(t, s.rec);
+    t->jobTag = s.tag;
+    t->tagReserve = 0;
+    myEpoch = s.epoch;
+    parity = t->chainParity;
+    first = 0;
+    t->succ.attached = false;
+    t->succAdopted++;
+    t->chainLaunches = had;
+  } else {
+    if (int rca = abandon_successor(t)) return rca;
+    t->maskSet ^= 1;
+    if (int rcm = wait_mask_merge(t, t->maskSet)) return rcm;
+    use_summary_record(t, t->sumRec ^ 1);
+    t->h_summary->done = 0;
+    t->h_summary->seq = 0;
+    t->h_summary->exhausted = 0;
+    myEpoch = ++c->enqEpoch;
+    t->jobTag = ((t->tagReserve ? t->tagReserve : t->jobTag) % 0x7FFFF) + 1;
+    t->tagReserve = 0;
+  }
+  t->spec.wasGoodSide = mask_side_set(t, t->maskSet);
   const TrackSummary* S = t->h_summary;
-  const long long myEpoch = ++c->enqEpoch;
-  int budget = 12;
+  const bool mayAttach = t->succession && c->pipeline && t->spinWait && t->enqueueHook && job.trackFrameSemantics;
+  int budget = 12, front = 0;
   if (t->recent[0] > 0) {
     budget = 0;
-    for (int i = 0; i < 4; i++) if (t->recent[i] > budget) budget = t->recent[i];
-    budget += t->budgetExtra;
+    int fewest = t->recent[0];
+    for (int i = 0; i < 4; i++) { if (t->recent[i] > budget) budget = t->recent[i]; if (t->recent[i] > 0 && t->recent[i] < fewest) fewest = t->recent[i]; }
+    budget += mayAttach ? t->budgetExtraSucc : t->budgetExtra;
+    front = fewest - 1;
   }
   if (t->budgetFixed > 0) budget = t->budgetFixed;
+  if (!mayAttach || t->budgetFixed > 0 || front <= 0) front = budget;
+  if (had > 0) {
+    budget -= had; front -= had;
+    if (front < 1) front = 1;
+    if (budget < front + 1) budget = front + 1;
+    if (t->budgetFixed > 0) front = budget = t->budgetFixed;
+  }
+  if (front > budget) front = budget;
   const bool sample = c->prof_on && ((c->prof_tick++ & 7) == 0);
 #ifdef LSD_DEVTOOLS
   t->dbgJobs++;
 #endif
-  t->jobTag = (t->jobTag % 0x7FFFF) + 1;
   t->launchOrdinal = 0;
-  t->h_summary->seq = 0;
-  t->h_summary->exhausted = 0;
   int guard = 0;
-  int parity = 0, first = 1;
   if (int rc = prof_collect(c)) return rc;
   lsdhip_host_mark(2);
   while (true) {
     if (sample) HIPCHK(hipEventRecord(c->ev_a, c->stream));
     int rc = LSDHIP_OK;
-    rc = launch_steps(t, job, budget, &parity, &first);
+    if (guard == 0) {
+      rc = launch_steps(t, job, front, &parity, &first, front == budget);
+      if (rc) return rc;
+      lsdhip_host_mark(3);
+      if (t->enqueueHook && job.trackFrameSemantics) t->enqueueHook(t->enqueueHookUser);
+      if (mayAttach) attach_successor(t, job, topLevel);
+      t->succOffer = nullptr;
+      if (budget > front) rc = launch_steps(t, job, budget - front, &parity, &first);
+    } else {
+      rc = launch_steps(t, job, budget, &parity, &first);
+    }
     if (rc) return rc;
     if (sample) { HIPCHK(hipEventRecord(c->ev_b, c->stream)); c->prof_pending = true; }
-    lsdhip_host_mark(3);
-    if (guard == 0 && t->enqueueHook && job.trackFrameSemantics) t->enqueueHook(t->enqueueHookUser);
     lsdhip_host_mark(4);
 #ifdef LSD_DEVTOOLS
     const auto tw0 = std::chrono::steady_clock::now();
@@ -1822,6 +2017,8 @@
     if (int rc2 = prof_collect(c)) return rc2;
     if (t->jobKf && t->jobKf->depthVersion != t->jobKfVersion && guard < 8) {
       t->jobKfVersion = t->jobKf->depthVersion;
+      if (int rca = abandon_successor(t)) return rca;
+      job.succ = TrackSucc{};
       t->h_summary->done = 0;
       parity = 0; first = 1;
       budget = 12;
@@ -1849,6 +2046,10 @@
     }
   }
 #endif
+  t->chainParity = parity;
+  t->prevNeeded = S->numLaunches + 1;
+  memcpy(t->prevSuccT0, S->succT0, sizeof(t->prevSuccT0));
+  if (S->diverged) { if (int rca = abandon_successor(t)) return rca; }
   t->numLaunches = S->numLaunches;
   t->recent[3] = t->recent[2]; t->recent[2] = t->recent[1]; t->recent[1] = t->recent[0]; t->recent[0] = t->numLaunches;
   for (int l = 0; l < LSD_LEVELS; l++) t->levelEvaluations[l] = S->levelEvals[l];
@@ -2011,7 +2212,7 @@
   const lsdm::SE3fH referenceToFrame0 = referenceToFrame;
   lsd_trace_val(c, 26, frame->id, t->dbgCum / 400ull);
 #endif
-  rc = track_device(t, job, LSD_TRACK_MAX_LEVEL - 1, referenceToFrame, &referenceToFrame);
+  rc = track_device(t, job, LSD_TRACK_MAX_LEVEL - 1, referenceToFrame, &referenceToFrame, frame);
   if (rc != LSDHIP_OK && rc != LSDHIP_DIVERGED) { t->jobKf = nullptr; return rc; }
 #ifdef LSD_DEVTOOLS
   static const bool replay = getenv("LSDHIP_TRACK_REPLAY") != nullptr;
diff --git a/lsd_slam_amd/driver.py b/lsd_slam_amd/driver.py
--- a/lsd_slam_amd/driver.py
+++ b/lsd_slam_amd/driver.py
@@ -18,7 +18,7 @@
 
 EXPORTED_SYMBOLS = ["lsdloop_create", "lsdloop_destroy", "lsdloop_run", "lsdloop_get_stats", "lsdloop_reset_stats",
                     "lsdloop_copy_keyframe_planes", "lsdloop_set_keyframe_ring", "lsdloop_keyframes_exported", "lsdloop_ctx",
-                    "lsdloop_last_error", "lsdloop_keep_keyframes", "lsdloop_keyframe_log", "lsdloop_set_live_queue", "lsdloop_set_pipeline", "lsdloop_set_speculation", "lsdloop_observe_time", "lsdloop_comm_unique_id", "lsdloop_comm_init", "lsdloop_comm_destroy",
+                    "lsdloop_last_error", "lsdloop_keep_keyframes", "lsdloop_keyframe_log", "lsdloop_set_live_queue", "lsdloop_set_pipeline", "lsdloop_set_speculation", "lsdloop_run_frames", "lsdloop_set_succession", "lsdloop_succession_stats", "lsdloop_observe_time", "lsdloop_comm_unique_id", "lsdloop_comm_init", "lsdloop_comm_destroy",
                     "lsdloop_gather_keyframes", "lsdband_create", "lsdband_destroy", "lsdband_window_rows", "lsdband_layout", "lsdband_load",
                     "lsdband_get", "lsdband_comm_init", "lsdband_run", "lsdband_synchronize", "lsdband_halo_bytes_per_pass", "lsdband_set_packed_exchange", "lsdband_set_overlap", "lsdband_tile_runs", "lsdband_plan", "lsdband_ipc_init", "lsdband_ipc_connect", "lsdband_ipc_failed", "lsdloop_gather_counts", "lsdloop_ipc_init", "lsdloop_ipc_connect", "lsdloop_ipc_result", "lsdloop_observe_work",
                     "lsdloopbatch_create", "lsdloopbatch_destroy", "lsdloopbatch_run", "lsdloopbatch_get_stats", "lsdloopbatch_ctx", "lsdloopbatch_set_keyframe_phases", "lsdloopbatch_set_pipeline", "lsdloopbatch_set_coarse_min_jobs", "lsdloopbatch_dropped",
@@ -60,6 +60,12 @@
         L.lsdloop_set_pipeline.argtypes = [vp, i]
         L.lsdloop_set_speculation.restype = i
         L.lsdloop_set_speculation.argtypes = [vp, i, i]
+        L.lsdloop_run_frames.restype = i
+        L.lsdloop_run_frames.argtypes = [vp, vp, vp, i, vp, vp]
+        L.lsdloop_set_succession.restype = i
+        L.lsdloop_set_succession.argtypes = [vp, i]
+        L.lsdloop_succession_stats.restype = i
+        L.lsdloop_succession_stats.argtypes = [vp, vp]
         L.lsdloop_observe_time.restype = i
         L.lsdloop_observe_time.argtypes = [vp, vp, vp]
         L.lsdloop_observe_work.restype = i
@@ -251,6 +257,23 @@
         done = _check(self.L.lsdloop_run(self.h_, arr, n, int(stop_at_keyframe), poses.ctypes.data if want_poses else None))
         return done, (poses[:done] if want_poses else None)
 
+    def run_frames(self, image_ptrs, next_ptrs=None):
+        n = len(image_ptrs)
+        arr = (C.c_void_p * n)(*image_ptrs)
+        nxt = (C.c_void_p * n)(*next_ptrs) if next_ptrs is not None else None
+        poses = np.zeros((n, 7), np.float64)
+        per = np.zeros((n, 8), np.int64)
+        done = _check(self.L.lsdloop_run_frames(self.h_, arr, nxt, n, poses.ctypes.data, per.ctypes.data))
+        return done, poses[:done], per[:done]
+
+    def set_succession(self, on=True):
+        _check(self.L.lsdloop_set_succession(self.h_, int(bool(on))))
+
+    def succession_stats(self):
+        out = np.zeros(4, np.int64)
+        _check(self.L.lsdloop_succession_stats(self.h_, out.ctypes.data))
+        return tuple(int(v) for v in out)
+
     def stats(self):
         s = LoopStats()
         _check(self.L.lsdloop_get_stats(self.h_, C.byref(s)))
diff --git a/lsd_slam_amd/driver/slam_loop.cpp b/lsd_slam_amd/driver/slam_loop.cpp
--- a/lsd_slam_amd/driver/slam_loop.cpp
+++ b/lsd_slam_amd/driver/slam_loop.cpp
@@ -282,7 +282,8 @@
   }
 }
 
-extern "C" int lsdloop_run(lsdloop* l, const uint8_t* const* images, int n, int stop_at_keyframe, double* out7) {
+static int run_frames(lsdloop* l, const uint8_t* const* images, const uint8_t* const* next_images, int n, int stop_at_keyframe, double* out7,
+                      long long* per_frame) {
   if (!l || !images || n < 0) return LSDHIP_E_ARG;
   try {
     int done = 0;
@@ -297,7 +298,14 @@
       const long drop0 = L.numDropped;
       long lev0[5];
       for (int k = 0; k < 5; k++) lev0[k] = L.levelEvaluations[k];
-      SE3 est = L.step(images[i], [](double) {}, (prefetch && i + 1 < n) ? images[i + 1] : nullptr);
+      const uint8_t* next = next_images ? next_images[i] : ((prefetch && i + 1 < n) ? images[i + 1] : nullptr);
+      SE3 est = L.step(images[i], [](double) {}, next);
+      if (per_frame) {
+        long long* o = per_frame + 8 * (size_t)i;
+        o[0] = L.evaluations - ev0; o[1] = L.launches - la0;
+        for (int k = 0; k < 5; k++) o[2 + k] = L.levelEvaluations[k] - lev0[k];
+        o[7] = L.numDropped - drop0;
+      }
       l->st.frames++;
       l->st.updates += L.numUpdates - updSeen;
       updSeen = L.numUpdates;
@@ -326,6 +334,25 @@
     g_err = e.what();
     return LSDHIP_E_STATE;
   }
+}
+extern "C" int lsdloop_run(lsdloop* l, const uint8_t* const* images, int n, int stop_at_keyframe, double* out7) {
+  return run_frames(l, images, nullptr, n, stop_at_keyframe, out7, nullptr);
+}
+extern "C" int lsdloop_run_frames(lsdloop* l, const uint8_t* const* images, const uint8_t* const* next_images, int n, double* out7, long long* per_frame) {
+  return run_frames(l, images, next_images, n, 0, out7, per_frame);
+}
+extern "C" int lsdloop_set_succession(lsdloop* l, int on) {
+  if (!l) return LSDHIP_E_ARG;
+  try { l->loop->tracker.setSuccession(on != 0); return LSDHIP_OK; }
+  catch (const Error& e) { g_err = e.what(); return e.status; }
+}
+extern "C" int lsdloop_succession_stats(lsdloop* l, long long out[4]) {
+  if (!l || !out) return LSDHIP_E_ARG;
+  try {
+    const SE3Tracker::SuccessionStats s = l->loop->tracker.successionStats();
+    out[0] = s.attached; out[1] = s.adopted; out[2] = s.abandoned; out[3] = s.on ? 1 : 0;
+    return LSDHIP_OK;
+  } catch (const Error& e) { g_err = e.what(); return e.status; }
 }
 extern "C" int lsdloop_get_stats(lsdloop* l, lsdloop_stats* out) {
   if (!l || !out) return LSDHIP_E_ARG;
```
